# david-gimeno/tailored-avsr

Measured on AMD Instinct MI355X. Metric: utterances/sec fwd+bwd, 12L tailored AV-Branchformer (Conv3d+ResNet-18 lip frontend, fusion, CTC+6L decoder), 4 s clips, batch 32/GPU, higher is better.
Workload: dtype f32

## Files before the change

include/tavsr.h:

```cpp
#ifndef TAVSR_H_
#define TAVSR_H_

#include <stdint.h>

#ifdef __cplusplus
extern "C" {
#endif

typedef void* tavsr_stream_t;

enum { TAVSR_OK = 0, TAVSR_EINVAL = -1, TAVSR_EALIGN = -2, TAVSR_EUNSUPPORTED = -3 };
enum { TAVSR_ACT_NONE = 0, TAVSR_ACT_RELU = 1, TAVSR_ACT_SWISH = 2, TAVSR_ACT_GELU = 3,
       TAVSR_ACT_TANH = 4, TAVSR_ACT_HARDTANH = 5, TAVSR_ACT_SELU = 6 };

int tavsr_version(void);
const char* tavsr_last_error_string(void);

int tavsr_spin(float us, tavsr_stream_t stream);
int tavsr_race_probe(float us, int mode);
int tavsr_stream_create(tavsr_stream_t* out);
int tavsr_probe_launch(int32_t kind, int32_t grid, int32_t block, float* buf, int64_t n, tavsr_stream_t stream);
int tavsr_probe_seam(int32_t kind, int32_t grid, int64_t per_wg, int32_t nphase, float* buf, void* ctl, uint32_t epoch0,
                     tavsr_stream_t stream);
int tavsr_mfma_peak_f32(int32_t iters, int32_t blocks, float* sink, tavsr_stream_t stream);
// ... 314 lines not shown
                         tavsr_stream_t stream);
int tavsr_merge_proj_ok(int32_t T, int32_t D);
int tavsr_merge_proj_fwd(const float* x1, const float* x2, const int64_t* lens, const int64_t* lens2, const float* const* params,
                         const float* w, const float* bias, const float* res, float alpha, float p_drop, const uint64_t* seed_dev,
                         uint64_t drop_offset, float* dots, float* score, float* wout, float* mix, float* out, int32_t B, int32_t T,
                         int32_t D, tavsr_stream_t stream);
int tavsr_merge_proj_fwd_dots(const float* x1, const float* x2, const int64_t* lens, const int64_t* lens2, const float* const* params,
                              const float* w, const float* bias, const float* res, float alpha, float p_drop, const uint64_t* seed_dev,
                              uint64_t drop_offset, const float* rowdots1, const float* rowdots2, float* dots, float* score, float* wout,
                              float* mix, float* out, int32_t B, int32_t T, int32_t D, tavsr_stream_t stream);
int64_t tavsr_merge_bwd_ws(int32_t B, int32_t D);
int tavsr_merge_bwd(const float* dm, const float* x1, const float* x2, const int64_t* lens, const int64_t* lens2,
                    const float* const* params, const float* score, const float* pooled, const float* w,
                    float* dx1, float* dx2, float* const* dparams, int32_t accumulate, float* ws, int32_t B,
                    int32_t T, int32_t D, tavsr_stream_t stream);

int tavsr_conv1_fwd(const float* x, const float* w, const float* bias, float* y, int32_t B, int32_t T,
                    int32_t F, int32_t C, tavsr_stream_t stream);
int64_t tavsr_conv1_bwd_ws(int32_t B, int32_t T, int32_t F, int32_t C);
int tavsr_conv1_bwd(const float* dz, const float* x, float* dw, float* db, int32_t accumulate, float* ws,
                    int32_t B, int32_t T, int32_t F, int32_t C, tavsr_stream_t stream);
int tavsr_im2col3x3s2(const float* y, float* col, int32_t B, int32_t Ti, int32_t Fi, int32_t C,
                      tavsr_stream_t stream);
int tavsr_col2im3x3s2_relu(const float* dcol, const float* yrelu, float* dz, int32_t B, int32_t Ti,
                           int32_t Fi, int32_t C, tavsr_stream_t stream);
int tavsr_transpose_inner(const float* in, float* out, int64_t nb, int32_t R, int32_t Cc, int32_t accumulate,
                          tavsr_stream_t stream);
int tavsr_utterance_mvn(const float* x, const int64_t* lens, float* y, int32_t B, int32_t T, int32_t F,
                        tavsr_stream_t stream);

int64_t tavsr_ctc_loss_ws(int32_t B, int32_t T, int32_t Lmax);
int tavsr_ctc_loss(const float* logits, int64_t ld_t, int64_t ld_b, const int64_t* hlens,
                   const int64_t* targets, int64_t ld_tgt, const int64_t* tlens, int32_t blank,
                   int32_t zero_infinity, float* loss, float* grad, float* ws, int32_t B, int32_t T,
                   int32_t V, int32_t Lmax, tavsr_stream_t stream);
int tavsr_ctc_greedy(const float* logits, int64_t ld_t, int64_t ld_b, const int64_t* hlens, int32_t blank,
                     int64_t* ids, int64_t* hyp, int64_t* hyp_len, int32_t B, int32_t T, int32_t V,
                     tavsr_stream_t stream);
int tavsr_ctc_align_lds_ok(int32_t T, int32_t Lmax);
int64_t tavsr_ctc_align_ws(int32_t N, int32_t T, int32_t Lmax);
int tavsr_ctc_align(const float* logits, int64_t ld_t, int64_t ld_b, const int64_t* hlens, const int32_t* rows,
                    const int64_t* targets, int64_t ld_tgt, const int64_t* tlens, int32_t blank, int64_t* align,
                    float* frame_lp, int32_t* span, float* score, void* ws, int32_t N, int32_t T, int32_t V, int32_t Lmax,
                    tavsr_stream_t stream);

int tavsr_lstm_rows_per_wg(void);
int tavsr_lstm_wt(const float* w_hh, float* w_hh_t, int32_t H, tavsr_stream_t stream);
int tavsr_lstm_fwd(const float* xg, int64_t ld_xg, const float* w_hh_t, const float* b_ih, const float* b_hh,
                   const float* h0, const float* c0, const int64_t* lens, float* y, float* hprev, float* c_all,
                   float* gates, float* hN, float* cN, int32_t B, int32_t L, int32_t H, tavsr_stream_t stream);
int tavsr_lstm_bwd(const float* dy, const float* dhN, const float* dcN, const float* w_hh, const float* c0,
                   const int64_t* lens, const float* c_all, const float* gates, float* dgates, float* dh0, float* dc0,
                   int32_t B, int32_t L, int32_t H, tavsr_stream_t stream);
int tavsr_lstm_step(const float* xg, int64_t ld_xg, const float* w_hh_t, const float* b_ih, const float* b_hh,
                    const float* h_in, const float* c_in, const uint8_t* commit, float* h_out, float* c_out, int32_t N,
                    int32_t H, tavsr_stream_t stream);
int tavsr_rnnt_mask_rows(const float* x, const int64_t* lens, int32_t extra, float* out, int32_t B, int32_t Tn, int32_t D,
                         tavsr_stream_t stream);
int64_t tavsr_rnnt_ws(int32_t B, int32_t T, int32_t U1, int32_t J, int32_t V, int32_t chunk, int32_t grad);
int tavsr_rnnt_joint_rows(const float* e, const float* d, const float* w_out, const float* b_out, const int32_t* y,
                          int64_t ld_y, const int64_t* tlens, const int64_t* ulens, int32_t blank, float* lse,
                          float* lp_blank, float* lp_label, float* ws, int32_t B, int32_t T, int32_t U1, int32_t J,
                          int32_t V, int32_t chunk, tavsr_stream_t stream);
int tavsr_rnnt_lattice_lds_ok(int32_t T, int32_t U1);
int64_t tavsr_rnnt_lattice_ws(int32_t B, int32_t T, int32_t U1);
int tavsr_rnnt_lattice(const float* lp_blank, const float* lp_label, const int64_t* tlens, const int64_t* ulens, float* nll,
                       float* occ, float* p_blank, float* p_label, float* ws, int32_t B, int32_t T, int32_t U1,
                       tavsr_stream_t stream);
int tavsr_rnnt_joint_grad(const float* e, const float* d, const float* w_out, const float* b_out, const int32_t* y,
                          int64_t ld_y, const int64_t* tlens, const int64_t* ulens, int32_t blank, const float* lse,
                          const float* occ, const float* p_blank, const float* p_label, const float* gscale, float inv_b,
                          float* de, float* dd, float* dw_out, float* db_out, float* ws, int32_t B, int32_t T, int32_t U1,
                          int32_t J, int32_t V, int32_t chunk, tavsr_stream_t stream);
int tavsr_rnnt_frame_z(const float* e, const float* d, const int32_t* frame, float* z, int32_t B, int32_t T, int32_t J,
                       tavsr_stream_t stream);
int tavsr_rnnt_greedy_pick(const float* logits, int64_t ldv, const int64_t* tlens, int32_t blank, int32_t* frame,
                           int64_t* tok, uint8_t* commit, int64_t* hyp, int64_t ld_hyp, int32_t* hyp_len, float* score,
                           int32_t B, int32_t V, tavsr_stream_t stream);

int tavsr_rnnt_search_ok(int32_t kind, int32_t K, int32_t V, int32_t T, int32_t u_max, int32_t max_sym_exp);
int64_t tavsr_rnnt_search_ws(int32_t kind, int32_t K, int32_t T, int32_t u_max, int32_t max_sym_exp);
int32_t tavsr_rnnt_search_ws_offset(int32_t kind, int32_t K, int32_t T, int32_t u_max, int32_t max_sym_exp, int32_t which);
int tavsr_rnnt_search_init(int32_t* ws, const int64_t* tlens, int32_t* row_t, int32_t U, int32_t kind, int32_t K, int32_t V,
                           int32_t T, int32_t u_max, int32_t max_sym_exp, tavsr_stream_t stream);
int tavsr_rnnt_search_z(const float* e, const float* d, const int32_t* row_t, float* z, int32_t N, int32_t K, int32_t T,
                        int32_t J, tavsr_stream_t stream);
int tavsr_rnnt_row_topk(const float* logits, int64_t ldv, const int32_t* row_t, float* lp_blank, float* topv, int32_t* topi,
                        int32_t N, int32_t V, int32_t K, tavsr_stream_t stream);
int tavsr_rnnt_gather_state(const float* src_h, const float* src_c, const int32_t* idx, float* dst_h, float* dst_c, int32_t L,
                            int32_t Ns, int32_t Nd, int32_t H, tavsr_stream_t stream);
int tavsr_rnnt_alsd_step(int32_t* ws, const int64_t* tlens, const float* lp_blank, const float* topv, const int32_t* topi,
                         int32_t* row_t, int32_t* parent, int64_t* tok, uint8_t* commit, int32_t U, int32_t K, int32_t V,
                         int32_t T, int32_t u_max, tavsr_stream_t stream);
int tavsr_rnnt_tsd_step(int32_t* ws, const int64_t* tlens, const float* lp_blank, const float* topv, const int32_t* topi,
                        int32_t* row_t, int32_t* parent, int64_t* tok, uint8_t* commit, int32_t* a_src, int32_t* b_sel,
                        int32_t v, int32_t U, int32_t K, int32_t V, int32_t T, int32_t max_sym_exp, tavsr_stream_t stream);

int tavsr_maskctc_init(const float* logits, int64_t ld_t, int64_t ld_b, const int64_t* hlens, int32_t blank,
                       int32_t mask_token, double threshold, int32_t n_iterations, int64_t* y_in, int64_t* y_hat,
                       float* tok_prob, int64_t ld_y, int64_t* y_len, int32_t* plan, int32_t B, int32_t T, int32_t V,
                       tavsr_stream_t stream);
int tavsr_maskctc_step(const float* logits, int64_t ld_l, int64_t ld_b, int64_t* y_in, int64_t ld_y,
                       const int64_t* y_len, const int32_t* plan, int32_t it, int32_t mask_token, int32_t B, int32_t L,
                       int32_t V1, tavsr_stream_t stream);

enum { TAVSR_MASK_UNIFORM_MAX_L = 4096 };
int tavsr_mask_uniform(const int64_t* text, int64_t ld_text, int32_t B, int32_t Lmax, int32_t mask_token, int32_t eos,
                       int32_t ignore_id, const uint64_t* seed_dev, uint64_t offset, int64_t* ys_in, int64_t* ys_out,
                       int64_t ld_y, int32_t* n_target, tavsr_stream_t stream);
int tavsr_count_recip(const int32_t* n, int32_t B, float* inv, tavsr_stream_t stream);

int tavsr_lm_shift(const int64_t* text, int64_t ld_text, const int64_t* lengths, int32_t B, int32_t W, int32_t sos_eos,
                   int64_t* x, int64_t* t, int64_t ld_y, int32_t Wout, int64_t* x_lengths, int32_t* n, tavsr_stream_t stream);
int tavsr_lm_row_sums(const float* x, int64_t ldx, float* out, int32_t rows, int32_t cols, tavsr_stream_t stream);

int tavsr_lsm_loss(const float* logits, int64_t ld, const int64_t* target, int32_t ignore, float smoothing,
                   float* row_loss, float* grad, int32_t* correct, int64_t rows, int32_t V,
                   tavsr_stream_t stream);
int tavsr_embed_pe(const int64_t* ids, const float* table, const float* pe, float scale, float* out, int64_t N,
                   int32_t L, int32_t D, tavsr_stream_t stream);
int tavsr_embed_pe_step(const int64_t* ids, const float* table, const float* pe, float scale, float* out, int64_t N,
                        int32_t L, int32_t D, const int32_t* step_dev, tavsr_stream_t stream);
int tavsr_embed_bwd(const int64_t* ids, const float* dout, float scale, float* dtable, int64_t N, int32_t V,
                    int32_t D, int32_t accumulate, tavsr_stream_t stream);

int tavsr_im2col2d(const float* x, float* col, int64_t N, int32_t H, int32_t W, int32_t C, int32_t KH, int32_t KW,
                   int32_t stride, int32_t pad, tavsr_stream_t stream);
int tavsr_col2im2d(const float* dcol, float* dx, int64_t N, int32_t H, int32_t W, int32_t C, int32_t KH, int32_t KW,
                   int32_t stride, int32_t pad, const float* extra, tavsr_stream_t stream);
int tavsr_im2col_stem(const float* x, float* col, int32_t B, int32_t T, int32_t H, int32_t W, tavsr_stream_t stream);
int64_t tavsr_bn_ws(int64_t M, int32_t C);
int tavsr_bn_stats(const float* x, int64_t M, int32_t C, float eps, float momentum, float* mean, float* var, float* rstd,
                   float* running_mean, float* running_var, int64_t* num_batches_tracked, float* ws, tavsr_stream_t stream);
int tavsr_bn_apply_fwd(const float* x, const float* mean, const float* rstd, const float* gamma, const float* beta,
                       const float* res, float* y, int64_t M, int32_t C, int32_t act, tavsr_stream_t stream);
int tavsr_bn_bwd(const float* dy, const float* x, const float* mean, const float* rstd, const float* gamma, const float* beta,
                 const float* res, float* dz, float* dx, float* dgamma, float* dbeta, int64_t M, int32_t C, int32_t act,
                 float* ws, tavsr_stream_t stream);
int tavsr_bn_bwd_pooled(const float* dpool, const uint8_t* idx, const float* x, const float* mean, const float* rstd,
                        const float* gamma, const float* beta, float* dx, float* dgamma, float* dbeta, int64_t N, int32_t H,
                        int32_t W, int32_t C, int32_t act, float* ws, tavsr_stream_t stream);
int tavsr_rsqrt_eps(const float* v, float eps, float* out, int64_t n, tavsr_stream_t stream);
int tavsr_maxpool3x3s2_fwd(const float* x, float* y, uint8_t* idx, int64_t N, int32_t H, int32_t W, int32_t C,
                           tavsr_stream_t stream);
int tavsr_bn_act_maxpool3x3s2_fwd(const float* x, const float* mean, const float* rstd, const float* gamma, const float* beta,
                                  int32_t act, float* y, uint8_t* idx, int64_t N, int32_t H, int32_t W, int32_t C,
                                  tavsr_stream_t stream);
int tavsr_maxpool3x3s2_bwd(const float* dy, const uint8_t* idx, float* dx, int64_t N, int32_t H, int32_t W, int32_t C,
                           tavsr_stream_t stream);
int tavsr_avgpool_fwd(const float* x, float* y, int64_t N, int32_t P, int32_t C, tavsr_stream_t stream);
int tavsr_avgpool_bwd(const float* dy, float* dx, int64_t N, int32_t P, int32_t C, tavsr_stream_t stream);
int tavsr_fill(float* p, float value, int64_t n, tavsr_stream_t stream);
int tavsr_conv_wflip(const float* w2d, float* wflip, int32_t Cout, int32_t Cin, tavsr_stream_t stream);
int tavsr_copy2d(const float* src, int64_t lds, float* dst, int64_t ldd, int64_t M, int64_t N, tavsr_stream_t stream);

int tavsr_stft_frames(const float* wav, const float* window, float* frames, int32_t B, int64_t N, int32_t T, int32_t n_fft,
                      int32_t hop, int32_t center, tavsr_stream_t stream);
int tavsr_power_spec(const float* spec, int64_t ld_spec, float* P, int32_t ldp, int32_t nfreq, int32_t B, int32_t T,
                     const int64_t* olens, tavsr_stream_t stream);
int tavsr_log_mask(const float* mel, float* out, int32_t B, int32_t T, int32_t n_mels, const int64_t* olens, float floor_,
                   tavsr_stream_t stream);
int tavsr_time_warp(const float* x, float* y, int32_t B, int32_t T, int32_t F, const int64_t* center, const int64_t* warped,
                    const int64_t* lens, tavsr_stream_t stream);
int tavsr_specaug_mask(float* x, int32_t B, int32_t T, int32_t F, const int64_t* fpos, const int64_t* flen, int32_t nf,
                       const int64_t* tpos, const int64_t* tlen, int32_t nt, tavsr_stream_t stream);

int tavsr_rowlin(const float* x, int64_t ldx, const int64_t* gather, const float* gamma, const float* beta, float eps,
                 const float* W, int64_t ldw, const float* bias, int32_t act, const float* res, int64_t ldr,
                 const int64_t* res_gather, float* out, int64_t ldo, int32_t N, int32_t K, int32_t Nout, tavsr_stream_t stream);
int tavsr_rowlin_parts(const float* x, int64_t ldx, int32_t x_parts, int64_t x_pstride, const float* gamma, const float* beta,
                       float eps, const float* W, int64_t ldw, const float* bias, int32_t act, const float* res, int64_t ldr,
                       int32_t res_parts, int64_t res_pstride, float* out, int64_t ldo, int32_t ksplit, int64_t out_pstride,
                       int32_t N, int32_t K, int32_t Nout, tavsr_stream_t stream);
int tavsr_tree_attn_tune(int32_t mode);
int tavsr_rowlin_ok(int32_t N, int32_t K, int32_t with_ln, int32_t ksplit);
int tavsr_tree_attn_step(const float* q, int64_t ldq, const float* kpool, const float* vpool, int64_t ldkv,
                         const int32_t* anc, int64_t ld_anc, int32_t nkeys, float* out, int64_t ldo, int32_t N, int32_t H,
                         int32_t dk, float scale, const int32_t* step_dev, const float* k_new, const float* v_new,
                         int32_t group, tavsr_stream_t stream);
int tavsr_kv_append(const float* k, const float* v, int64_t ld_src, float* kpool, float* vpool, int64_t ldkv, int32_t N,
                    int32_t D, int32_t max_steps, const int32_t* step_dev, tavsr_stream_t stream);
int tavsr_ctc_prefix_step(const float* logp, const int64_t* lens, const float* r_prev, const float* s_prev,
                          const int64_t* last_tok, const int64_t* cand, float* r_new, float* psi, float* psi_abs, float* eos,
                          float* eos_abs, int32_t N, int32_t K, int32_t T, int32_t V, int32_t C, int32_t out_len,
                          int32_t blank, const int32_t* step_dev, tavsr_stream_t stream);
int tavsr_ctc_prefix_step_topk(const float* logp, const int64_t* lens, const float* r_prev, const float* s_prev,
                               const int64_t* last_tok, const float* full, int64_t* cand, float* r_new, float* psi, float* psi_abs,
                               float* eos, float* eos_abs, int32_t N, int32_t K, int32_t T, int32_t V, int32_t C, int32_t out_len,
                               int32_t blank, const int32_t* step_dev, tavsr_stream_t stream);
int tavsr_log_softmax_rows(const float* x, int64_t ldx, float* y, int64_t ldy, int32_t M, int32_t V, float alpha, float add,
                           int32_t accumulate, tavsr_stream_t stream);
int tavsr_beam_combine(const float* full, const int64_t* cand, const float* psi, float* psi_abs, const float* eos_s,
                       const float* eos_abs, const float* s_prev, const float* score, float* weighted, int32_t N, int32_t V,
                       int32_t C, int32_t eos, float w_ctc, tavsr_stream_t stream);
int tavsr_beam_combine_topk(const float* full, const int64_t* cand, const float* psi, float* psi_abs, const float* eos_s,
                            const float* eos_abs, const float* s_prev, const float* score, float* weighted, float* top_s,
                            int64_t* top_i, int32_t N, int32_t K, int32_t V, int32_t C, int32_t eos, float w_ctc,
                            tavsr_stream_t stream);
int tavsr_beam_select_topk(const float* dec, const float* z_lm, float w_lm, float add, const float* psi_all, float* psi_abs_all,
                           const float* eos_s, const float* eos_abs, const float* s_prev, const float* score, float* full_out,
                           float* weighted, int64_t* cand_out, float* top_s, int64_t* top_i, int32_t N, int32_t K, int32_t V,
                           int32_t C, int32_t eos, float w_ctc, tavsr_stream_t stream);
int tavsr_beam_reorder(const int64_t* top_i, const float* top_s, const int64_t* cand, const float* r_new, const float* psi_abs,
                       const int64_t* yseq, const int32_t* anc, float* r_out, float* s_out, int64_t* yseq_out, int32_t* anc_out,
                       int64_t* tok_out, float* score_out, int32_t N, int32_t K, int32_t V, int32_t C, int32_t T, int32_t ld_y,
                       int32_t ld_a, const int32_t* step_dev, int32_t* hist, int32_t hist_steps, tavsr_stream_t stream);
int tavsr_beam_reorder_begin(const int64_t* top_i, const float* top_s, const int64_t* cand, const float* r_new, const float* psi_abs,
                             const int64_t* yseq, const int32_t* anc, float* r_out, float* s_out, int64_t* yseq_out, int32_t* anc_out,
                             int64_t* tok_out, float* score_out, int32_t N, int32_t K, int32_t V, int32_t C, int32_t T, int32_t ld_y,
                             int32_t ld_a, const int32_t* step_dev, int32_t* hist, int32_t hist_steps, const int32_t* maxlen,
                             int32_t eos, tavsr_stream_t stream);
int tavsr_beam_step_begin(float* score, const int64_t* tok, int32_t* anc, int32_t ld_a, const int32_t* maxlen, int32_t N, int32_t K,
                          int32_t eos, const int32_t* step_dev, tavsr_stream_t stream);
int tavsr_ctc_beam_search_ok(int32_t K, int32_t V, int32_t T);
int tavsr_ctc_beam_search(const float* logp, const int64_t* lens, const int32_t* maxlen, int32_t* hist, int32_t* n_steps, int32_t U,
                          int32_t K, int32_t T, int32_t V, int32_t hist_steps, int32_t sos, int32_t eos, int32_t blank, float w_ctc,
                          float add, int32_t end_detect, float d_end, tavsr_stream_t stream);
int tavsr_timesync_ok(int32_t K, int32_t V, int32_t T, int32_t C);
int64_t tavsr_timesync_ws(int32_t K, int32_t V, int32_t T, int32_t C);
int32_t tavsr_timesync_ws_offset(int32_t K, int32_t V, int32_t T, int32_t C, int32_t which);
int tavsr_timesync_init(int32_t* ws, int64_t* tok, int32_t* pos, int32_t* nkeys, int32_t* anc, int64_t ld_anc, int32_t* frame_dev,
                        int32_t U, int32_t K, int32_t V, int32_t T, int32_t C, int32_t sos, int32_t blank, tavsr_stream_t stream);
int tavsr_timesync_step(const float* lpz, const int64_t* lens, int32_t* ws, const float* dec_new, float* dec_rows,
                        const float* lm_new, float* lm_rows, int64_t* tok, int32_t* pos, int32_t* nkeys, int32_t* anc,
                        int32_t* anc_tmp, int64_t ld_anc, const int32_t* frame_dev, int32_t U, int32_t K, int32_t V, int32_t T,
                        int32_t C, int32_t sos, int32_t blank, float w_ctc, float w_dec, float w_lm, float pen,
                        tavsr_stream_t stream);
int tavsr_timesync_search(const float* lpz, const int64_t* lens, int32_t* ws, int32_t U, int32_t K, int32_t V, int32_t T, int32_t C,
                          int32_t sos, int32_t blank, float w_ctc, float pen, tavsr_stream_t stream);
int tavsr_tree_attn_rows(const float* q, int64_t ldq, const float* kpool, const float* vpool, int64_t ldkv, const int32_t* anc,
                         int64_t ld_anc, const int32_t* nkeys_row, int32_t max_keys, float* out, int64_t ldo, int32_t N, int32_t H,
                         int32_t dk, float scale, const float* k_new, const float* v_new, tavsr_stream_t stream);
int tavsr_embed_pe_rows(const int64_t* ids, const float* table, const float* pe, float scale, float* out, int64_t N, int32_t L,
                        int32_t D, const int32_t* pos, tavsr_stream_t stream);
enum { TAVSR_NGRAM_MAX_ORDER = 8 };
int tavsr_ngram_score(const int32_t* word, const float* logp, const float* backoff, const int32_t* child_begin, int32_t n_unigrams,
                      int32_t order, int32_t bos_word, float unk_logp, const int32_t* word_map, const int64_t* yseq, int64_t ld_y,
                      int32_t L, int32_t step, const int32_t* step_dev, const int64_t* cand, int32_t C, float alpha, float add,
                      int32_t accumulate, float* out, int64_t ldo, int32_t N, int32_t V, tavsr_stream_t stream);
int tavsr_act_fwd(const float* x, float* y, int64_t n, int32_t act, tavsr_stream_t stream);

int tavsr_adam_step(float* p, const float* g, float* m, float* v, int64_t n, float lr, float beta1, float beta2, float eps,
                    int64_t step, float grad_scale, tavsr_stream_t stream);
int tavsr_adamw_step(float* p, const float* g, float* m, float* v, int64_t n, float lr, float beta1, float beta2, float eps,
                     float weight_decay, int64_t step, float grad_scale, tavsr_stream_t stream);

int tavsr_bucket_copy(float* const* ptrs_dev, const int64_t* off_dev, const int64_t* n_dev, int32_t ntensors, float* flat,
                      float scale, int32_t to_flat, int64_t max_n, tavsr_stream_t stream);

int tavsr_dp_unique_id(void* id128);
int tavsr_dp_init(int32_t rank, int32_t nranks, const void* id128);
int32_t tavsr_dp_world(void);
int tavsr_dp_allreduce(float* flat, int64_t n, tavsr_stream_t stream);
int tavsr_dp_broadcast(float* flat, int64_t n, int32_t root, tavsr_stream_t stream);
int tavsr_dp_destroy(void);

int tavsr_multi_add(float* const* dst, const float* const* src, const int64_t* n, int32_t ntensors, tavsr_stream_t stream);
int tavsr_multi_copy(void* const* dst, const void* const* src, const int64_t* nbytes, int32_t nbuffers, tavsr_stream_t stream);
int tavsr_multi_copy_inc(void* const* dst, const void* const* src, const int64_t* nbytes, int32_t nbuffers, int64_t* counters,
                         int32_t ncounters, tavsr_stream_t stream);

int tavsr_dropout(const float* x, float* y, int64_t n, float p, const uint64_t* seed_dev, uint64_t offset,
                  tavsr_stream_t stream);
int tavsr_rng_advance(uint64_t* seed_dev, tavsr_stream_t stream);
int tavsr_rng_step(uint64_t* seed_dev, uint64_t* step_seed_dev, tavsr_stream_t stream);
int tavsr_dropout_add(const float* a, const float* t, float* y, int64_t n, float p, float alpha, const uint64_t* seed_dev,
                      uint64_t offset, tavsr_stream_t stream);
int tavsr_dropout_act_bwd(const float* dh, const float* z, float* dz, int64_t n, float p, int32_t act,
                          const uint64_t* seed_dev, uint64_t offset, tavsr_stream_t stream);

int tavsr_edit_distance(const int32_t* ref, const int64_t* ref_off, const int32_t* hyp, const int64_t* hyp_off, int32_t n_pairs,
                        int32_t max_len, int32_t* dist, tavsr_stream_t stream);
int tavsr_bootstrap_rates(const int32_t* dist, const int32_t* reflen, int32_t n, int32_t iters, uint64_t seed, double* rates,
                          tavsr_stream_t stream);

int tavsr_video_prep(const void* src, int32_t is_u8, int32_t Ts, int32_t H, int32_t W, const int32_t* frames, int32_t T,
                     int32_t y0, int32_t x0, int32_t th, int32_t tw, int32_t flip, const float* mean, const float* std,
                     int32_t n_affine, const uint8_t* masked, float* mean_frame_ws, float* dst, int32_t Tpad, float pad,
                     tavsr_stream_t stream);
int tavsr_add_noise(const float* audio, const float* noise, float* out, int64_t n, float inv_snr, tavsr_stream_t stream);
int64_t tavsr_resample_len(int64_t n_in, double factor);
int tavsr_resample_sinc(const float* x, int64_t n_in, float* y, int64_t n_out, double factor, double rolloff, int32_t zeros, double beta,
                        tavsr_stream_t stream);

#ifdef __cplusplus
}
#endif
#endif
```

tailored-avsr_amd/csrc/gemm_conv.hip:

```cpp
#include <algorithm>
#include <vector>

#include "gemm_glds.h"

namespace tavsr {

constexpr int kOrdRuns = 80;
struct TileOrder {
  int nruns;
  int start[kOrdRuns];
  int cum[kOrdRuns + 1];
  int w[kOrdRuns];
};

__host__ __device__ inline void tile_order_map(const TileOrder& o, int b, int tiles_m, int tiles_n, int& mt, int& nt) {
  const int per = 8 * tiles_n;
  const int g = b / per, j = b - g * per, s0 = 8 * g;
  int r0 = 0;
  while (r0 + 1 < o.nruns && o.cum[r0 + 1] <= s0) ++r0;
  bool uniform = s0 + 8 <= tiles_m;
  if (uniform) {
    int r7 = r0;
    while (r7 + 1 < o.nruns && o.cum[r7 + 1] <= s0 + 7) ++r7;
    uniform = o.w[r7] == o.w[r0];
  }
  const int s = s0 + (uniform ? (j & 7) : j / tiles_n);
  nt = uniform ? (j >> 3) : j % tiles_n;
  int r = r0;
  while (r + 1 < o.nruns && o.cum[r + 1] <= s) ++r;
  mt = o.start[r] + s - o.cum[r];
}

__host__ __device__ inline int dw_tile_order(int q, int tiles_m, int tiles_n, int H, int W) {
  if (tiles_n % 9 != 0) return q;
  const int tpt = tiles_n / 9, per = tiles_m * tpt;
  const int rank = q / per, rem = q - rank * per;
  const unsigned long long taps = (H - 1) * W >= H * (W - 1) ? 0x862053714ull : 0x862071534ull;
  const int tap = (int)((taps >> (4 * rank)) & 15);
  return (rem / tpt) * tiles_n + tap * tpt + rem % tpt;
}

__host__ __device__ inline void dw_xcd_order(int j, int tiles_m, int tiles_n, int ns, int& zs, int& q) {
  const int tiles = tiles_m * tiles_n;
  zs = j / tiles;
  q = j - zs * tiles;
  if (tiles_n % 9 != 0) return;
  const int per = tiles_m * (tiles_n / 9);
  const int rank = j / (ns * per), rem = j - rank * (ns * per);
  zs = rem / per;
  q = rank * per + rem - zs * per;
}

struct ConvGeom {
  int cs, p0, Ho, Wo;
  bool c9;
  __device__ __forceinline__ explicit ConvGeom(const tavsr_gemm_desc& d) {
    cs = d.conv_stride > 1 ? d.conv_stride : 1;
    c9 = d.conv_taps != 1;
    p0 = d.conv_taps == 90 ? 1 : 0;
    Ho = (d.conv_H - 1 - 2 * p0) / cs + 1;
    Wo = (d.conv_W - 1 - 2 * p0) / cs + 1;
  }
};

template <int BM, int NT>
struct ImageRows {
  using L = GLoader<BM, false, NT>;
  int64_t off[L::NR];
  uint32_t mask[L::NR];
  __device__ __forceinline__ void issue(const TileCtx& c, bool c9, int kk, int tap, float* img) const {
    const tavsr_gemm_desc& d = c.d;
    const int toff = c9 ? (tap / 3 - 1) * d.conv_W + (tap % 3 - 1) : 0;
    const int64_t delta = (int64_t)toff * d.conv_C + (kk - tap * d.conv_C);
#pragma unroll
    for (int i = 0; i < L::NR; ++i)
      dma16(((mask[i] >> tap) & 1u) ? c.A + off[i] + delta : d.conv_zero, img + (i * NT + c.wave * 64) * 4);
  }
};

template <int BM, int NT>
struct ConvRowsA {
  using R = ImageRows<BM, NT>;
  static constexpr int kDma = R::L::NR;
  const TileCtx& c;
  bool c9;
  R rows;
  __device__ __forceinline__ explicit ConvRowsA(const TileCtx& c_) : c(c_) {
    const tavsr_gemm_desc& d = c.d;
    const ConvGeom g(d);
    c9 = g.c9;
    R::L::offsets(d.lda, c.m0, d.M, c.tid, rows.off);
#pragma unroll
    for (int i = 0; i < R::L::NR; ++i) {
      const int m = min(c.m0 + ((i * NT + c.tid) >> 3), d.M - 1);
      const int x = (m % g.Wo) * g.cs + g.p0, y = ((m / g.Wo) % g.Ho) * g.cs + g.p0;
      if (g.cs > 1 || g.p0) rows.off[i] += ((int64_t)((m / (g.Wo * g.Ho)) * d.conv_H + y) * d.conv_W + x - m) * d.conv_C;
      uint32_t mk = 0;
#pragma unroll
      for (int tap = 0; tap < 9; ++tap)
        mk |= (uint32_t)((unsigned)(y + tap / 3 - 1) < (unsigned)d.conv_H && (unsigned)(x + tap % 3 - 1) < (unsigned)d.conv_W) << tap;
      rows.mask[i] = g.c9 ? mk : 1u;
    }
  }
  __device__ __forceinline__ void issue(int kt, float* img) {
    const int kk = c.kbeg + kt * kBK;
    rows.issue(c, c9, kk, kk / c.d.conv_C, img);
  }
};
template <int BM, int BN, int NT, bool BKM>
struct SourceFor<1, false, BM, BN, NT, false, BKM> {
  using type = PairSource<ConvRowsA<BM, NT>, PlainOperand<BN, BKM, NT, true>, BM>;
};

template <int BM, int BN, int NT, bool BKM>
struct PosMajorRowsSource : SourceDefaults {
  using R = ImageRows<BM, NT>;
  using LB = GLoader<BN, BKM, NT>;
  static constexpr int kDma = R::L::NR + LB::NR;
  static constexpr bool kPosMajorRows = true;
  const TileCtx& c;
  PosMajor pm{};
  uint32_t taps = 0;
  int tap, cb, nk;
  bool c9;
  R rows;
  int64_t offB[LB::NR];
  __device__ __forceinline__ explicit PosMajorRowsSource(const TileCtx& c_) : c(c_) {
    const tavsr_gemm_desc& d = c.d;
    const ConvGeom g(d);
    c9 = g.c9;
    LB::offsets(d.ldb, c.n0, d.N, c.tid, offB);
    pm.H = g.Ho; pm.W = g.Wo;
    pm.st = g.cs; pm.HI = d.conv_H; pm.WI = d.conv_W;
    pm.n = d.M / (g.Ho * g.Wo);
    const int vlo = c.m0 / pm.n, vhi = min(c.m0 + BM - 1, d.M - 1) / pm.n;
    for (int v = vlo; v <= vhi; ++v) {
      int y, x;
      pm.pos(v, y, x);
      taps |= pm.taps(y, x);
      pm.rp = y * g.Wo + x;
    }
    pm.uni = vlo == vhi;
    pm.base = vlo * pm.n;
    nk = 0;
    for (int t = 0; t < 9; ++t) {
      const int lo = max(c.kbeg, t * d.conv_C), hi = min(c.kend, (t + 1) * d.conv_C);
      if (((taps >> t) & 1u) && hi > lo) nk += (hi - lo) / kBK;
    }
    tap = c.kbeg / d.conv_C;
    cb = (c.kbeg - tap * d.conv_C) / kBK;
    if (!((taps >> tap) & 1u)) {
      const uint32_t up = taps >> (tap + 1) << (tap + 1);
      tap = up ? __builtin_ctz(up) : 9;
      cb = 0;
    }
#pragma unroll
    for (int i = 0; i < R::L::NR; ++i) {
      const int q = i * NT + c.tid, row = q >> 3;
      const int r = min(c.m0 + row, d.M - 1);
      int y, x, img;
      if (pm.uni) {
        y = pm.rp / g.Wo; x = pm.rp - y * g.Wo; img = r - pm.base;
      } else {
        const int v = r / pm.n;
        pm.pos(v, y, x);
        img = r - v * pm.n;
      }
      rows.off[i] = ((int64_t)img * (d.conv_H * d.conv_W) + g.cs * y * d.conv_W + g.cs * x) * d.lda + ((q & 7) ^ ((row >> 1) & 7)) * 4;
      rows.mask[i] = pm.taps(y, x);
    }
  }
  __device__ __forceinline__ int steps() const { return nk; }
  __device__ __forceinline__ const PosMajor* row_map() const { return &pm; }
  __device__ __forceinline__ void issue(int, float* stage) {
    const tavsr_gemm_desc& d = c.d;
    const int ktap = tap, kk = tap * d.conv_C + cb * kBK;
    const int wrap = (cb + 1) * kBK >= d.conv_C;
    const uint32_t up = taps >> (tap + 1) << (tap + 1);
    cb = wrap ? 0 : cb + 1;
    tap = !wrap ? tap : up ? __builtin_ctz(up) : 9;
    rows.issue(c, c9, kk, ktap, stage);
    LB::issue(c.B + (BKM ? (int64_t)kk * d.ldb : kk), offB, stage + BM * kBK, c.wave);
  }
};
template <int BM, int BN, int NT, bool BKM>
struct SourceFor<1, true, BM, BN, NT, false, BKM> {
  using type = PosMajorRowsSource<BM, BN, NT, BKM>;
};

template <int BN, int NT>
struct PatchB {
  using L = GLoader<BN, true, NT>;
  static constexpr int kDma = L::NR;
  const TileCtx& c;
  const ConvGeom g;
  int ox[L::NR], oy[L::NR], img[L::NR];
  int sb, salo, sahi, tapoff, cb, dy, dx;
  __device__ __forceinline__ explicit PatchB(const TileCtx& c_) : c(c_), g(c_.d) {
    const tavsr_gemm_desc& d = c.d;
    const int sa = kBK / g.Wo;
    sb = kBK - sa * g.Wo;
    sahi = sa / g.Ho;
    salo = sa - sahi * g.Ho;
    const int tap = c.n0 / d.conv_C;
    cb = c.n0 - tap * d.conv_C;
    dy = g.c9 ? tap / 3 - 1 : 0;
    dx = g.c9 ? tap % 3 - 1 : 0;
    tapoff = dy * d.conv_W + dx;
#pragma unroll
    for (int i = 0; i < L::NR; ++i) {
      const int m = c.kbeg + (i * NT + c.tid) / (BN / 4);
      const int t = m / g.Wo;
      ox[i] = m - t * g.Wo;
      img[i] = t / g.Ho;
      oy[i] = t - img[i] * g.Ho;
    }
  }
  __device__ __forceinline__ void issue(int, float* dst) {
    const tavsr_gemm_desc& d = c.d;
#pragma unroll
    for (int i = 0; i < L::NR; ++i) {
      const int r = (((i * NT + c.tid) % (BN / 4)) * 4);
      const int x = ox[i] * g.cs + g.p0, y = oy[i] * g.cs + g.p0;
      const bool ok = (unsigned)(y + dy) < (unsigned)d.conv_H && (unsigned)(x + dx) < (unsigned)d.conv_W;
      const int64_t pix = (int64_t)(img[i] * d.conv_H + y) * d.conv_W + x;
      dma16(ok ? c.B + (pix + tapoff) * d.conv_C + cb + r : d.conv_zero, dst + (i * NT + c.wave * 64) * 4);
      int nx = ox[i] + sb;
      const int w1 = nx >= g.Wo ? 1 : 0;
      nx -= w1 ? g.Wo : 0;
      int ny = oy[i] + salo + w1;
      const int w2 = ny >= g.Ho ? 1 : 0;
      ny -= w2 ? g.Ho : 0;
      ox[i] = nx; oy[i] = ny; img[i] += sahi + w2;
    }
  }
};
template <int BM, int BN, int NT>
struct SourceFor<2, false, BM, BN, NT, true, true> {
  using type = PairSource<PlainOperand<BM, true, NT, false>, PatchB<BN, NT>, BM>;
};

template <int BM, int BN, int NT>
struct PatchWalkSource : SourceDefaults {
  using LA = GLoader<BM, true, NT>;
  using LB = GLoader<BN, true, NT>;
  static constexpr int kDma = LA::NR + LB::NR;
  const TileCtx& c;
  const ConvGeom g;
  int64_t offA[LA::NR];
  int tapoff, cb, dy, dx;
  int n, i0, nk;
  int v = 0, img = 0, x = 0, y = 0;
  __device__ __forceinline__ static int rowsum_n0(const tavsr_gemm_desc& d) { return 4 * d.conv_C; }
  __device__ __forceinline__ bool ok(int py, int px) const {
    return (unsigned)(g.cs * py + dy) < (unsigned)c.d.conv_H && (unsigned)(g.cs * px + dx) < (unsigned)c.d.conv_W;
  }
  __device__ __forceinline__ explicit PatchWalkSource(const TileCtx& c_) : c(c_), g(c_.d) {
    const tavsr_gemm_desc& d = c.d;
    const int tap = c.n0 / d.conv_C;
    cb = c.n0 - tap * d.conv_C;
    dy = g.c9 ? tap / 3 - 1 : 0;
    dx = g.c9 ? tap % 3 - 1 : 0;
    tapoff = dy * d.conv_W + dx;
    const int P = g.Ho * g.Wo;
    i0 = c.kbeg / P;
    n = (c.kend - c.kbeg) / P;
    LA::offsets(d.lda, c.m0, d.M, c.tid, offA);
#pragma unroll
    for (int i = 0; i < LA::NR; ++i) offA[i] -= (int64_t)((i * NT + c.tid) / (BM / 4)) * d.lda;
    if (n % kBK == 0) {
      int ny = 0, nx = 0;
      for (int py = 0; py < g.Ho; ++py) ny += (unsigned)(g.cs * py + dy) < (unsigned)d.conv_H;
      for (int px = 0; px < g.Wo; ++px) nx += (unsigned)(g.cs * px + dx) < (unsigned)d.conv_W;
      nk = (n / kBK) * ny * nx;
    } else {
      nk = 0;
      int prev = 0, py = 0, px = 0;
      for (int pv = 0; pv < P; ++pv) {
        if (ok(py, px)) {
          const int s_lo = max(pv * n / kBK, prev), s_hi = ((pv + 1) * n - 1) / kBK + 1;
          if (s_hi > s_lo) { nk += s_hi - s_lo; prev = s_hi; }
        }
        if (++px == g.Wo) { px = 0; ++py; }
      }
    }
  }
  __device__ __forceinline__ int steps() const { return nk; }
  __device__ __forceinline__ void advance() {
    img += kBK;
    while (img >= n) {
      img -= n;
      ++v;
      if (++x == g.Wo) { x = 0; ++y; }
    }
  }
  __device__ __forceinline__ int64_t locate(int kl, int& py, int& px, int& pimg) const {
    int pv = v;
    pimg = img + kl;
    py = y; px = x;
    while (pimg >= n) {
      pimg -= n;
      ++pv;
      if (++px == g.Wo) { px = 0; ++py; }
    }
    pimg += i0;
    return (int64_t)pimg * (g.Ho * g.Wo) + pv;
  }
  __device__ __forceinline__ void issue(int, float* stage) {
    const tavsr_gemm_desc& d = c.d;
    for (;;) {
      bool any = false;
      int end = img + kBK, py = y, px = x;
      for (;;) {
        any |= ok(py, px);
        if (end <= n) break;
        end -= n;
        if (++px == g.Wo) { px = 0; ++py; }
      }
      if (any) break;
      advance();
    }
#pragma unroll
    for (int i = 0; i < LA::NR; ++i) {
      int py, px, pimg;
      const int64_t pix = locate((i * NT + c.tid) / (BM / 4), py, px, pimg);
      dma16(c.A + pix * d.lda + offA[i], stage + (i * NT + c.wave * 64) * 4);
    }
#pragma unroll
    for (int i = 0; i < LB::NR; ++i) {
      const int r = (((i * NT + c.tid) % (BN / 4)) * 4);
      int py, px, pimg;
      locate((i * NT + c.tid) / (BN / 4), py, px, pimg);
      const int64_t pix = ((int64_t)pimg * d.conv_H + g.cs * py) * d.conv_W + g.cs * px;
      dma16(ok(py, px) ? c.B + (pix + tapoff) * d.conv_C + cb + r : d.conv_zero, stage + BM * kBK + (i * NT + c.wave * 64) * 4);
    }
    advance();
  }
};
template <int BM, int BN, int NT>
struct SourceFor<2, true, BM, BN, NT, true, true> {
// ... 80 lines not shown
    const int ft = m / (g.Wo * g.Ho);
    t = ft % g.T;
    off = (ft * g.H + 2 * ho) * g.W + 2 * wo;
    th = frame_row_ok();
  }
  __device__ __forceinline__ void issue(int, float* img) {
#pragma unroll
    for (int i = 0; i < kDma; ++i) {
      const bool ok = th && (unsigned)(2 * wo + c3) < (unsigned)g.W;
      dma4(ok ? c.B + (off + tapoff) : c.d.conv_zero, img + i * NT + c.wave * 64);
      wo += 4;
      off += 8;
      if (wo >= g.Wo) {
        wo -= g.Wo;
        off += g.W;
        if (++ho == g.Ho) {
          ho = 0;
          if (++t == g.T) t = 0;
        }
        th = frame_row_ok();
      }
    }
  }
};
template <int BM, int BN, int NT>
struct SourceFor<5, false, BM, BN, NT, true, true> {
  using type = PairSource<PlainOperand<BM, true, NT, false>, Stem5B<BN, NT>, BM>;
};

struct PaddedStemGeom {
  int Hp, Wp, Tp, Ho, Wo, T;
  __device__ __forceinline__ explicit PaddedStemGeom(const tavsr_gemm_desc& d)
      : Hp(d.conv_H), Wp(d.conv_W), Tp(d.conv_C), Ho((d.conv_H - 6) / 2), Wo((d.conv_W - 8) / 2), T(d.conv_C - 5) {}
  __device__ __forceinline__ int pixel(int m) const {
    const int wo = m % Wo, ho = (m / Wo) % Ho, ft = m / (Wo * Ho);
    return (((ft / T) * Tp + ft % T) * Hp + 2 * ho) * Wp + 2 * wo;
  }
};

template <int BM, int NT>
struct Stem6A {
  using L = GLoader<BM, false, NT>;
  static constexpr int kDma = L::NR;
  const TileCtx& c;
  const PaddedStemGeom g;
  int base[L::NR], cl[L::NR];
  __device__ __forceinline__ explicit Stem6A(const TileCtx& c_) : c(c_), g(c_.d) {
#pragma unroll
    for (int i = 0; i < L::NR; ++i) {
      const int q = i * NT + c.tid, row = q >> 3;
      cl[i] = (q & 7) ^ ((row >> 1) & 7);
      base[i] = g.pixel(min(c.m0 + row, c.d.M - 1));
    }
  }
  __device__ __forceinline__ void issue(int kt, float* img) {
#pragma unroll
    for (int i = 0; i < L::NR; ++i) {
      const int ch = (c.kbeg >> 2) + kt * 8 + cl[i], r = ch >> 1, a = r / 7, b = r - 7 * a;
      dma16(c.A + (base[i] + (a * g.Hp + b) * g.Wp + 4 * (ch & 1)), img + (i * NT + c.wave * 64) * 4);
    }
  }
};
template <int BM, int BN, int NT>
struct SourceFor<6, false, BM, BN, NT, false, false> {
  using type = PairSource<Stem6A<BM, NT>, PlainOperand<BN, false, NT, true>, BM>;
};

template <int BN, int NT>
struct Stem7B {
  using L = GLoader<BN, true, NT>;
  static constexpr int kDma = L::NR;
  const TileCtx& c;
  const PaddedStemGeom g;
  int wo[L::NR], ho[L::NR], t[L::NR], off[L::NR];
  int tapoff;
  __device__ __forceinline__ explicit Stem7B(const TileCtx& c_) : c(c_), g(c_.d) {
    constexpr int CPR = BN / 4;
    int ch = (c.n0 >> 2) + (c.tid % CPR);
    if (ch >= 72) ch = 0;
    const int r = ch >> 1, a = r / 7, b = r - 7 * a;
    tapoff = (a * g.Hp + b) * g.Wp + 4 * (ch & 1);
#pragma unroll
    for (int i = 0; i < L::NR; ++i) {
      const int m = c.kbeg + (i * NT + c.tid) / CPR;
      wo[i] = m % g.Wo; ho[i] = (m / g.Wo) % g.Ho; t[i] = (m / (g.Wo * g.Ho)) % g.T;
      off[i] = g.pixel(m);
    }
  }
  __device__ __forceinline__ void issue(int, float* img) {
    constexpr int STEP = 32;
#pragma unroll
    for (int i = 0; i < L::NR; ++i) {
      dma16(c.B + (off[i] + tapoff), img + (i * NT + c.wave * 64) * 4);
      wo[i] += STEP;
      off[i] += 2 * STEP;
      while (wo[i] >= g.Wo) {
        wo[i] -= g.Wo;
        off[i] += 2 * g.Wp - 2 * g.Wo;
        if (++ho[i] == g.Ho) {
          ho[i] = 0;
          off[i] += (g.Hp - 2 * g.Ho) * g.Wp;
          if (++t[i] == g.T) { t[i] = 0; off[i] += (g.Tp - g.T) * g.Hp * g.Wp; }
        }
      }
    }
  }
};
template <int BM, int BN, int NT>
struct SourceFor<7, false, BM, BN, NT, true, true> {
  using type = PairSource<PlainOperand<BM, true, NT, false>, Stem7B<BN, NT>, BM>;
};

struct GemmArgsOrd {
  GemmArgs g;
  TileOrder ord;
};
template <int CONV, bool PM>
struct TileMap<CONV, PM, true> {
  __device__ __forceinline__ static const GemmArgs& map(const GemmArgsOrd& x, int& bid, int& zidx) {
    bid = xcd_remap(blockIdx.x, gridDim.x);
    zidx = blockIdx.z;
    if (x.ord.nruns > 0) {
      int mt, nt;
      tile_order_map(x.ord, blockIdx.x, x.g.tiles_m, x.g.tiles_n, mt, nt);
      bid = mt * x.g.tiles_n + nt;
    }
    return x.g;
  }
  __device__ __forceinline__ static const GemmArgs& map(const GemmArgs& args, int& bid, int& zidx) {
    bid = xcd_remap(blockIdx.x, gridDim.x);
    zidx = blockIdx.z;
    if (args.zmap) {
      const int tiles = gridDim.x, l = blockIdx.x + tiles * blockIdx.z, j = l >> 3;
      int zs = j / tiles;
      bid = j % tiles;
      if constexpr (PM && CONV == 2) {
        if (!(args.d.conv_posmajor & 2)) {
          if (args.n_big > 0) dw_xcd_order(j, args.tiles_m, args.tiles_n, args.nsplit >> 3, zs, bid);
          bid = dw_tile_order(bid, args.tiles_m, args.tiles_n, args.d.conv_H, args.d.conv_W);
        }
      }
      zidx = (l & 7) + 8 * zs;
    }
    return args;
  }
};

static int conv_ho(const tavsr_gemm_desc& d) { return (d.conv_H - 1) / std::max(d.conv_stride, 1) + 1; }
static int conv_wo(const tavsr_gemm_desc& d) { return (d.conv_W - 1) / std::max(d.conv_stride, 1) + 1; }

constexpr int kPmStride2MaxPos = 36;
static bool conv_pm(const tavsr_gemm_desc& d) {
  const bool stride_ok = d.conv_stride <= 1 || (d.conv_stride == 2 && (d.conv_posmajor & 8) && conv_ho(d) * conv_wo(d) <= kPmStride2MaxPos);
  return d.conv_posmajor && (d.conv_mode == 1 || d.conv_mode == 2) && stride_ok && (d.conv_taps == 0 || d.conv_taps == 9) &&
         (d.conv_mode == 2 || !d.a_rowsum);
}

static void tile_order_build(const tavsr_gemm_desc& d, int BM, int nsplit, TileOrder& o) {
  o.nruns = 0;
  const int cs = std::max(d.conv_stride, 1);
  const int P = conv_ho(d) * conv_wo(d);
  if (nsplit != 1 || (d.conv_posmajor & 2) || P <= 0 || d.M < P) return;
  struct Key { int H, W, cs, M, BM; };
  static thread_local Key last{0, 0, 0, 0, 0};
  static thread_local TileOrder last_o;
  if (last.H == d.conv_H && last.W == d.conv_W && last.cs == cs && last.M == d.M && last.BM == BM) { o = last_o; return; }
  PosMajor pm{};
  pm.H = conv_ho(d); pm.W = conv_wo(d); pm.n = d.M / P;
  pm.st = cs; pm.HI = d.conv_H; pm.WI = d.conv_W;
  std::vector<uint32_t> tp(P);
  for (int v = 0; v < P; ++v) {
    int y, x;
    pm.pos(v, y, x);
    tp[v] = pm.taps(y, x);
  }
  struct Run { int start, len, w; };
  std::vector<Run> runs;
  const int tiles_m = cdiv(d.M, BM);
  for (int i = 0; i < tiles_m; ++i) {
    const int vlo = (int)((int64_t)i * BM / pm.n);
    const int vhi = std::min((int)(std::min<int64_t>((int64_t)i * BM + BM - 1, d.M - 1) / pm.n), P - 1);
    uint32_t mk = 0;
    for (int v = vlo; v <= vhi; ++v) mk |= tp[v];
    const int w = __builtin_popcount(mk);
    if (!runs.empty() && runs.back().w == w) ++runs.back().len;
    else runs.push_back(Run{i, 1, w});
    if ((int)runs.size() > kOrdRuns) return;
  }
  std::stable_sort(runs.begin(), runs.end(), [](const Run& a, const Run& b) { return a.w > b.w; });
  int cum = 0;
  for (size_t r = 0; r < runs.size(); ++r) {
    o.start[r] = runs[r].start; o.cum[r] = cum; o.w[r] = runs[r].w;
    cum += runs[r].len;
  }
  o.cum[runs.size()] = cum;
  o.nruns = (int)runs.size();
  last = Key{d.conv_H, d.conv_W, cs, d.M, BM};
  last_o = o;
}

template <int BM, int BN, int MINW, bool AK, bool BKM, int CONV, bool PM>
static int launch_conv_tile(const tavsr_gemm_desc& d, const Plan& p, hipStream_t s) {
  const int zmap = (CONV == 2 || CONV == 5 || CONV == 7) && p.nsplit >= 8 && p.nsplit % 8 == 0;
  const bool two = PM && CONV == 2;
  GemmArgs a{d, p.kchunk, p.nsplit, cdiv(d.M, BM), cdiv(d.N, BN), (int)vec_epi_ok(d), zmap, two ? p.n_big : 0, two ? p.kunit : 0};
  const dim3 grid(a.tiles_m * a.tiles_n, 1, p.nsplit);
  if constexpr (PM && CONV == 1) {
    GemmArgsOrd ao{a, {}};
    tile_order_build(d, BM, p.nsplit, ao.ord);
    hipLaunchKernelGGL((gemm_glds_kernel<BM, BN, 2, 2, 2, MINW, AK, BKM, 1, CONV, true>), grid, dim3(256), 0, s, ao);
  } else {
    hipLaunchKernelGGL((gemm_glds_kernel<BM, BN, 2, 2, 2, MINW, AK, BKM, 1, CONV, PM>), grid, dim3(256), 0, s, a);
  }
  TAVSR_LAUNCH_CHECK();
  return launch_epilogue(a, s);
}

template <int BM, int BN, int MINW, bool AK, bool BKM, int CONV>
static int launch_conv_pm(const tavsr_gemm_desc& d, const Plan& p, hipStream_t s) {
  return conv_pm(d) ? launch_conv_tile<BM, BN, MINW, AK, BKM, CONV, true>(d, p, s) : launch_conv_tile<BM, BN, MINW, AK, BKM, CONV, false>(d, p, s);
}

int launch_conv(const tavsr_gemm_desc& d, const Plan& p, hipStream_t s) {
  switch (d.conv_mode) {
    case 1:
      if (d.b_kmajor) return launch_conv_pm<64, 64, 5, false, true, 1>(d, p, s);
      if (p.nsplit == 1 && d.N % 128 == 0) return launch_conv_pm<64, 128, 3, false, false, 1>(d, p, s);
      return launch_conv_pm<64, 64, 5, false, false, 1>(d, p, s);
    case 2:
      if (d.M % 128 == 0) return launch_conv_pm<128, 64, 3, true, true, 2>(d, p, s);
      return launch_conv_pm<64, 64, 5, true, true, 2>(d, p, s);
    case 4: return launch_conv_tile<64, 64, 5, false, false, 4, false>(d, p, s);
    case 5: return launch_conv_tile<64, 64, 5, true, true, 5, false>(d, p, s);
    case 6: return launch_conv_tile<64, 64, 5, false, false, 6, false>(d, p, s);
    default: return launch_conv_tile<64, 64, 5, true, true, 7, false>(d, p, s);
  }
}

Plan plan_conv(const tavsr_gemm_desc& d, bool can_split, int force_split) {
  Plan pc = plan(d, can_split, true);
  if ((d.conv_mode == 2 || d.conv_mode == 5 || d.conv_mode == 7) && can_split) {
    const bool wide = d.conv_mode == 2 && d.M % 128 == 0;
    const long tiles = (long)cdiv(d.M, wide ? 128 : 64) * cdiv(d.N, 64);
    constexpr long target64 = 2560L;
    constexpr long target128 = 2304L;
    const long target = wide ? target128 : target64;
    int unit = 32;
    if (conv_pm(d)) {
      const int P = conv_ho(d) * conv_wo(d);
      int g = P, b = 32;
      while (b) { const int t = g % b; g = b; b = t; }
      unit = P / g * 32;
      if (pc.nsplit > 1) {
        pc.kchunk = cdiv(pc.kchunk, unit) * unit;
        pc.nsplit = cdiv(d.K, pc.kchunk);
      }
    }
    const long want = std::min<long>(std::max<long>(1, target / tiles), d.K / 512);
    if (want > pc.nsplit) {
      pc.kchunk = cdiv(cdiv(d.K, want), unit) * unit;
      pc.nsplit = cdiv(d.K, pc.kchunk);
    }
    if (pc.nsplit >= 16 && pc.nsplit % 8 != 0) {
      for (long w8 = pc.nsplit / 8 * 8; w8 >= 8; w8 -= 8) {
        const int kc = cdiv(cdiv(d.K, w8), unit) * unit;
        if (cdiv(d.K, kc) % 8 == 0) { pc.kchunk = kc; pc.nsplit = cdiv(d.K, kc); break; }
        if (w8 < pc.nsplit / 2) break;
      }
    }
    if (conv_pm(d) && d.conv_mode == 2 && !(d.conv_posmajor & 4) && d.K % unit == 0) {
      const long U = d.K / unit, round4 = (wide ? 768 : 1280) / 4;
      const long w = std::min<long>(force_split > 0 ? force_split : want, U) / 8 * 8;
      const bool missed = target - (long)pc.nsplit * tiles > round4, hits = target - w * tiles <= round4;
      if (w >= 8 && U % w != 0 && (force_split > 0 || (missed && hits))) {
        pc.nsplit = (int)w;
        pc.kchunk = (int)(U / w) * unit;
        pc.n_big = (int)(U % w);
        pc.kunit = unit;
      }
    }
  }
  return pc;
}

}

extern "C" int tavsr_conv_tile_order(int H, int W, int images, int bm, int tiles_n, int32_t* tile_m, int32_t* tile_n, int max_blocks) {
  using namespace tavsr;
  if (H <= 0 || W <= 0 || images <= 0 || bm <= 0 || tiles_n <= 0) return 0;
  tavsr_gemm_desc d{};
  d.conv_H = H; d.conv_W = W; d.M = images * H * W; d.conv_posmajor = 1;
  TileOrder o;
  tile_order_build(d, bm, 1, o);
  if (o.nruns == 0) return 0;
  const int tiles_m = cdiv(d.M, bm), nwg = tiles_m * tiles_n;
  for (int b = 0; b < nwg && b < max_blocks; ++b) tile_order_map(o, b, tiles_m, tiles_n, tile_m[b], tile_n[b]);
  return nwg;
}

extern "C" int tavsr_conv_dw_tile_order(int H, int W, int tiles_m, int tiles_n, int32_t* tile, int max_tiles) {
  if (H <= 0 || W <= 0 || tiles_m <= 0 || tiles_n <= 0) return 0;
  for (int q = 0; q < tiles_m * tiles_n && q < max_tiles; ++q) tile[q] = tavsr::dw_tile_order(q, tiles_m, tiles_n, H, W);
  return tiles_m * tiles_n;
}

extern "C" int tavsr_conv_dw_plan(int H, int W, int cin, int cout, int images, int posmajor, int force_split, int32_t* out) {
  using namespace tavsr;
  if (H <= 0 || W <= 0 || cin <= 0 || cout <= 0 || images <= 0 || !out) return 0;
  tavsr_gemm_desc d{};
  d.conv_mode = 2; d.conv_H = H; d.conv_W = W; d.conv_C = cin; d.conv_stride = 1; d.conv_taps = 9; d.conv_posmajor = posmajor;
  d.M = cout; d.N = 9 * cin; d.K = images * H * W; d.a_kmajor = d.b_kmajor = 1; d.nb1 = d.nb2 = 1;
  const Plan p = plan_conv(d, true, force_split);
  out[0] = p.kchunk; out[1] = p.n_big; out[2] = p.kunit;
  return p.nsplit;
}

extern "C" int tavsr_conv_dw_xcd_order(int H, int W, int tiles_m, int tiles_n, int ns, int32_t* slice, int32_t* tile, int max_tiles) {
  if (H <= 0 || W <= 0 || tiles_m <= 0 || tiles_n <= 0 || ns <= 0) return 0;
  for (int j = 0; j < ns * tiles_m * tiles_n && j < max_tiles; ++j) {
    int zs, q;
    tavsr::dw_xcd_order(j, tiles_m, tiles_n, ns, zs, q);
    slice[j] = zs;
    tile[j] = tavsr::dw_tile_order(q, tiles_m, tiles_n, H, W);
  }
  return ns * tiles_m * tiles_n;
}

#ifdef TAVSR_GEMM_TRACE
namespace tavsr {
int conv_trace_read(unsigned long long* out, int max_rows) { return trace_read_unit(out, max_rows); }
}
#endif
```

tailored-avsr_amd/csrc/gemm_glds.h:

```cpp
#pragma once
#include <type_traits>

#include "common.h"

namespace tavsr {

typedef float f32x16 __attribute__((ext_vector_type(16)));
constexpr int kBK = 32;

struct GemmArgs {
  tavsr_gemm_desc d;
  int kchunk;
  int nsplit;
  int tiles_m, tiles_n;
  int vec_epi;
  int zmap;
  int n_big, kunit;
};

template <int ROWS, int BK, bool KMAJOR>
struct Tile {
  static constexpr int LD = KMAJOR ? (ROWS + 4) : (BK + 4);
  static constexpr int SIZE = KMAJOR ? BK * LD : ROWS * LD;
};
// ... 203 lines not shown
                                                int tid, int zidx, const PosMajor* pm = nullptr) {
  __syncthreads();
#pragma unroll
  for (int i = 0; i < TM; ++i)
#pragma unroll
    for (int j = 0; j < TN; ++j)
#pragma unroll
      for (int r = 0; r < 16; ++r)
        img[(wm * TM * 32 + i * 32 + (r & 3) + 8 * (r >> 2) + 4 * lk) * BN + wn * TN * 32 + j * 32 + lr] = acc[i][j][r];
  __syncthreads();
  constexpr int V4R = BN / 4, PER = BM * BN / 4 / NT;
  static_assert(BM * BN % (4 * NT) == 0, "tile must divide over the block");
  const bool split = nsplit > 1;
  float* base;
  int64_t ld;
  if (split) {
    base = d.ws + ((int64_t)zidx * gridDim.y + blockIdx.y) * ((int64_t)d.M * d.N);
    ld = d.N;
  } else {
    base = d.C + coff;
    ld = d.ldc;
  }
  const float* R = (!split && d.R) ? d.R + z1 * d.sR1 + z2 * d.sR2 : nullptr;
  float* Z = (!split && d.Z) ? d.Z + coff : nullptr;
  const float* DZ = (!split && d.DZ) ? d.DZ + coff : nullptr;
  const bool rowstat = BN == 64 && !split && d.rowstat != nullptr;
#pragma unroll
  for (int q = 0; q < PER; ++q) {
    const int idx = q * NT + tid, row = idx / V4R, c4 = idx % V4R;
    const int mv = m0 + row, n = n0 + 4 * c4;
    const bool ok = mv < d.M && n < d.N;
    const int m = PM && ok ? pm->row(mv) : mv;
    float4 v = make_float4(0.f, 0.f, 0.f, 0.f);
    if (ok) {
    v = *reinterpret_cast<const float4*>(img + row * BN + 4 * c4);
    const int64_t o = (int64_t)m * ld + n;
    if (!split) {
      if (d.bias) {
        const float4 b = *reinterpret_cast<const float4*>(d.bias + n);
        v.x += b.x; v.y += b.y; v.z += b.z; v.w += b.w;
      }
      if (Z) *reinterpret_cast<float4*>(Z + o) = v;
      v.x = act_fwd(d.act, v.x); v.y = act_fwd(d.act, v.y); v.z = act_fwd(d.act, v.z); v.w = act_fwd(d.act, v.w);
      if (DZ) {
        const float4 z = *reinterpret_cast<const float4*>(DZ + o);
        v.x *= act_bwd(d.dact, z.x); v.y *= act_bwd(d.dact, z.y); v.z *= act_bwd(d.dact, z.z); v.w *= act_bwd(d.dact, z.w);
      }
      if (d.drop_p > 0.f) {
        const uint64_t sd = d.drop_seed[0], ctr = (d.drop_offset >> 2) + (uint64_t)(((int64_t)m * d.N + n) >> 2);
        const uint32_t thr = (uint32_t)((double)d.drop_p * 4294967296.0);
        const float ik = 1.f / (1.f - d.drop_p);
        uint32_t w[4];
        philox4x32_10((uint32_t)ctr, (uint32_t)(ctr >> 32), 0u, 0u, (uint32_t)sd, (uint32_t)(sd >> 32), w);
        v.x = w[0] >= thr ? v.x * ik : 0.f; v.y = w[1] >= thr ? v.y * ik : 0.f;
        v.z = w[2] >= thr ? v.z * ik : 0.f; v.w = w[3] >= thr ? v.w * ik : 0.f;
      }
      v.x *= d.alpha; v.y *= d.alpha; v.z *= d.alpha; v.w *= d.alpha;
      if (R) {
        const float4 rr = *reinterpret_cast<const float4*>(R + (int64_t)m * d.ldr + n);
        v.x += rr.x; v.y += rr.y; v.z += rr.z; v.w += rr.w;
      }
    }
    *reinterpret_cast<float4*>(base + o) = v;
    }
    if (rowstat) {
      float s1 = ok ? (v.x + v.y) + (v.z + v.w) : 0.f, s2 = 0.f;
      if (d.rowdot_a) {
        const float4 wa = ok ? *reinterpret_cast<const float4*>(d.rowdot_a + n) : make_float4(0.f, 0.f, 0.f, 0.f);
        const float4 wb = ok ? *reinterpret_cast<const float4*>(d.rowdot_b + n) : make_float4(0.f, 0.f, 0.f, 0.f);
        s1 = (v.x * wa.x + v.y * wa.y) + (v.z * wa.z + v.w * wa.w);
        s2 = (v.x * wb.x + v.y * wb.y) + (v.z * wb.z + v.w * wb.w);
      }
#pragma unroll
      for (int o2 = 8; o2 > 0; o2 >>= 1) s1 += __shfl_xor(s1, o2, 64);
      if (!d.rowdot_a && ok) {
        const float tm = s1 / (float)min(64, d.N - n0);
        const float e0 = v.x - tm, e1 = v.y - tm, e2 = v.z - tm, e3 = v.w - tm;
        s2 = (e0 * e0 + e1 * e1) + (e2 * e2 + e3 * e3);
      }
#pragma unroll
      for (int o2 = 8; o2 > 0; o2 >>= 1) s2 += __shfl_xor(s2, o2, 64);
      if (c4 == 0 && mv < d.M)
        *reinterpret_cast<float2*>(d.rowstat + ((int64_t)m * ((d.N + 63) / 64) + n0 / 64) * 2) = make_float2(s1, s2);
    }
  }
}

static bool aligned16(const void* p) { return (reinterpret_cast<uintptr_t>(p) & 15) == 0; }
static bool vec_epi_ok(const tavsr_gemm_desc& d) {
  return d.N % 4 == 0 && d.ldc % 4 == 0 && d.sC1 % 4 == 0 && d.sC2 % 4 == 0 && aligned16(d.C) && (!d.bias || aligned16(d.bias)) &&
         (!d.Z || aligned16(d.Z)) && (!d.DZ || aligned16(d.DZ)) &&
         (!d.R || (aligned16(d.R) && d.ldr % 4 == 0 && d.sR1 % 4 == 0 && d.sR2 % 4 == 0)) && (!d.ws || aligned16(d.ws));
}

typedef __attribute__((address_space(3))) float lds_float;
typedef const __attribute__((address_space(1))) float glb_float;

template <int ROWS, bool KMAJOR, int NT>
struct GLoader {
  static constexpr int NR = ROWS * 8 / NT;
  static_assert(ROWS * 8 % NT == 0, "tile must divide over the block");
  __device__ static __forceinline__ void offsets(int64_t ld, int row0, int nrows, int tid, int64_t (&off)[NR]) {
#pragma unroll
    for (int i = 0; i < NR; ++i) {
      const int q = i * NT + tid;
      if (KMAJOR) {
        const int k = q / (ROWS / 4);
        int r = row0 + (q % (ROWS / 4)) * 4;
        if (r + 3 >= nrows) r = row0;
        off[i] = (int64_t)k * ld + r;
      } else {
        const int row = q >> 3, cp = q & 7;
        const int cl = cp ^ ((row >> 1) & 7);
        off[i] = (int64_t)min(row0 + row, nrows - 1) * ld + cl * 4;
      }
    }
  }
  __device__ static __forceinline__ void issue(const float* __restrict__ g, const int64_t (&off)[NR],
                                               float* __restrict__ stage, int wave) {
#pragma unroll
    for (int i = 0; i < NR; ++i)
      __builtin_amdgcn_global_load_lds((glb_float*)(g + off[i]), (lds_float*)(stage + (i * NT + wave * 64) * 4), 16, 0, 0);
  }
};

__device__ __forceinline__ void dma16(const float* src, float* dst) {
  __builtin_amdgcn_global_load_lds((glb_float*)src, (lds_float*)dst, 16, 0, 0);
}
__device__ __forceinline__ void dma4(const float* src, float* dst) {
  __builtin_amdgcn_global_load_lds((glb_float*)src, (lds_float*)dst, 4, 0, 0);
}

#ifndef TAVSR_GEMM_SB
#define TAVSR_GEMM_SB 1
#endif
#if TAVSR_GEMM_SB
#define GEMM_SB() __builtin_amdgcn_sched_barrier(0)
#else
#define GEMM_SB()
#endif

template <int ROWS, bool KMAJOR>
__device__ __forceinline__ void read_frag_g(const float* __restrict__ s, int row, int g, int lk, float (&f)[4]) {
  if (KMAJOR) {
    const float* p = s + (g * 8 + 4 * lk) * ROWS + row;
#pragma unroll
    for (int j = 0; j < 4; ++j) f[j] = p[j * ROWS];
  } else {
    const float4 v = *reinterpret_cast<const float4*>(s + row * 32 + (((2 * g + lk) ^ ((row >> 1) & 7)) << 2));
    f[0] = v.x; f[1] = v.y; f[2] = v.z; f[3] = v.w;
  }
}

template <int N>
__device__ __forceinline__ void wait_vmcnt() {
  asm volatile("s_waitcnt vmcnt(%0)" ::"n"(N) : "memory");
}

#ifdef TAVSR_GEMM_TRACE
constexpr int kTraceMax = 1 << 15;
static __device__ unsigned long long g_trace[kTraceMax][6];
static __device__ unsigned int g_trace_n;
#define TAVSR_TRACE_DECL unsigned long long tr_t[4], tr_c[4]; tr_t[0] = wall_clock64(); tr_t[1] = tr_t[0]; tr_c[1] = tr_c[2] = 0;
#define TAVSR_TRACE_AT(i) { tr_t[i] = wall_clock64(); tr_c[i] = __builtin_readcyclecounter(); }
static int trace_read_unit(unsigned long long* out, int max_rows) {
  unsigned int n = 0;
  if (hipDeviceSynchronize() != hipSuccess) return -1;
  if (hipMemcpyFromSymbol(&n, HIP_SYMBOL(g_trace_n), sizeof(n)) != hipSuccess) return -1;
  int rows = (int)(n < (unsigned)kTraceMax ? n : kTraceMax);
  if (rows > max_rows) rows = max_rows;
  if (rows > 0 && hipMemcpyFromSymbol(out, HIP_SYMBOL(g_trace), (size_t)rows * 6 * sizeof(unsigned long long)) != hipSuccess) return -1;
  n = 0;
  if (hipMemcpyToSymbol(HIP_SYMBOL(g_trace_n), &n, sizeof(n)) != hipSuccess) return -1;
  return rows;
}
int conv_trace_read(unsigned long long* out, int max_rows);
#else
#define TAVSR_TRACE_DECL
#define TAVSR_TRACE_AT(i)
#endif

struct TileCtx {
  const tavsr_gemm_desc& d;
  const float* A;
  const float* B;
  int m0, n0;
  int kbeg, kend;
  int tid, wave;
};

struct SourceDefaults {
  static constexpr bool kPosMajorRows = false;
  __device__ __forceinline__ const PosMajor* row_map() const { return nullptr; }
  __device__ __forceinline__ static int rowsum_n0(const tavsr_gemm_desc&) { return 0; }
  __device__ __forceinline__ void fix_last(float*, int, int, int) const {}
};

template <int ROWS, bool KMAJOR, int NT, bool B_SIDE>
struct PlainOperand {
  using L = GLoader<ROWS, KMAJOR, NT>;
  static constexpr int kDma = L::NR;
  const TileCtx& c;
  int64_t off[L::NR];
  const float* gk;
  int64_t kstep;
  __device__ __forceinline__ explicit PlainOperand(const TileCtx& c_) : c(c_) {
    const int64_t ld = B_SIDE ? c.d.ldb : c.d.lda;
    L::offsets(ld, B_SIDE ? c.n0 : c.m0, B_SIDE ? c.d.N : c.d.M, c.tid, off);
    kstep = KMAJOR ? (int64_t)kBK * ld : kBK;
    gk = (B_SIDE ? c.B : c.A) + (KMAJOR ? (int64_t)c.kbeg * ld : c.kbeg);
  }
  __device__ __forceinline__ void issue(int kt, float* img) { L::issue(gk + kt * kstep, off, img, c.wave); }
};

template <class HA, class HB, int BM>
struct PairSource : SourceDefaults {
  static constexpr int kDma = HA::kDma + HB::kDma;
  HA a;
  HB b;
  int nk;
  __device__ __forceinline__ explicit PairSource(const TileCtx& c) : a(c), b(c), nk((c.kend - c.kbeg) / kBK) {}
  __device__ __forceinline__ int steps() const { return nk; }
  __device__ __forceinline__ void issue(int kt, float* stage) {
    a.issue(kt, stage);
    b.issue(kt, stage + BM * kBK);
  }
};

template <int CONV, bool PM, int BM, int BN, int NT, bool AK, bool BKM>
struct SourceFor;
template <int BM, int BN, int NT, bool AK, bool BKM>
struct SourceFor<0, false, BM, BN, NT, AK, BKM> {
  using type = PairSource<PlainOperand<BM, AK, NT, false>, PlainOperand<BN, BKM, NT, true>, BM>;
};

template <int BM, int BN, int WM, int WN, int S, bool AK, bool BKM, int KW = 1, int CONV = 0, bool PM = false>
__device__ __forceinline__ void glds_tile(const tavsr_gemm_desc& d, int kchunk, int nsplit, int tiles_n, int bid, bool vec_epi,
                                          int zidx, int n_big = 0, int kunit = 0) {
  constexpr int BK = kBK, NG = BK / 8;
  static_assert(NG % KW == 0, "k-groups must divide over the wave sets");
  static_assert(!PM || KW == 1, "position-major order: one wave set");
  constexpr int NT = WM * WN * KW * 64;
  constexpr int TM = BM / WM / 32, TN = BN / WN / 32;
  using Src = typename SourceFor<CONV, PM, BM, BN, NT, AK, BKM>::type;
  constexpr int ASZ = BM * BK, STAGE = (BM + BN) * BK;
  constexpr int G = Src::kDma;
  static_assert((S - 2) * G <= 63, "vmcnt field");
  __shared__ __attribute__((aligned(1024))) float smem[S * STAGE];

  const int tid = threadIdx.x;
  const int lane = tid & 63;
  const int wave = __builtin_amdgcn_readfirstlane(tid >> 6);
  const int kw = wave / (WM * WN), w2 = wave % (WM * WN);
  const int wm = w2 / WN, wn = w2 % WN;
  const int lr = lane & 31, lk = lane >> 5;

  TAVSR_TRACE_DECL
  const int m0 = (bid / tiles_n) * BM;
  const int n0 = (bid % tiles_n) * BN;
  const int z1 = blockIdx.y / d.nb2, z2 = blockIdx.y % d.nb2;
  const float* A = d.A + z1 * d.sA1 + z2 * d.sA2;
  const float* B = d.B + z1 * d.sB1 + z2 * d.sB2;
  const int64_t coff = z1 * d.sC1 + z2 * d.sC2;

  f32x16 acc[TM][TN];
#pragma unroll
  for (int i = 0; i < TM; ++i)
#pragma unroll
    for (int j = 0; j < TN; ++j)
#pragma unroll
      for (int r = 0; r < 16; ++r) acc[i][j][r] = 0.f;
  float asum[TM];
#pragma unroll
  for (int i = 0; i < TM; ++i) asum[i] = 0.f;
  float bpre[TN];
#pragma unroll
  for (int j = 0; j < TN; ++j) {
    const int n = n0 + wn * TN * 32 + j * 32 + lr;
    bpre[j] = (d.bias && nsplit == 1 && n < d.N) ? d.bias[n] : 0.f;
  }

  const int kbeg = zidx * kchunk + min(zidx, n_big) * kunit;
  const int kend = min(d.K, kbeg + kchunk + (zidx < n_big ? kunit : 0));
  const TileCtx ctx{d, A, B, m0, n0, kbeg, kend, tid, wave};
  Src src(ctx);
  const int nk = src.steps();
  const bool want_rowsum = d.a_rowsum != nullptr && n0 == Src::rowsum_n0(d) && wn == 0;

  const int arow = wm * TM * 32 + lr, brow = wn * TN * 32 + lr;
  auto compute = [&](int st) {
    const float* a_s = smem + st * STAGE;
    const float* b_s = a_s + ASZ;
    float af[2][TM][4], bf[2][TN][4];
#pragma unroll
    for (int i = 0; i < TM; ++i) read_frag_g<BM, AK>(a_s, arow + i * 32, kw, lk, af[0][i]);
#pragma unroll
    for (int j = 0; j < TN; ++j) read_frag_g<BN, BKM>(b_s, brow + j * 32, kw, lk, bf[0][j]);
#pragma unroll
    for (int q = 0; q < NG / KW; ++q) {
      const int c = q & 1;
      if (q + 1 < NG / KW) {
#pragma unroll
        for (int i = 0; i < TM; ++i) read_frag_g<BM, AK>(a_s, arow + i * 32, kw + (q + 1) * KW, lk, af[c ^ 1][i]);
#pragma unroll
        for (int j = 0; j < TN; ++j) read_frag_g<BN, BKM>(b_s, brow + j * 32, kw + (q + 1) * KW, lk, bf[c ^ 1][j]);
      }
      GEMM_SB();
#pragma unroll
      for (int kk = 0; kk < 4; ++kk)
#pragma unroll
        for (int i = 0; i < TM; ++i)
#pragma unroll
          for (int j = 0; j < TN; ++j)
            acc[i][j] = __builtin_amdgcn_mfma_f32_32x32x2f32(af[c][i][kk], bf[c][j][kk], acc[i][j], 0, 0, 0);
#pragma unroll
      for (int i = 0; i < TM; ++i) asum[i] += (af[c][i][0] + af[c][i][1]) + (af[c][i][2] + af[c][i][3]);
      GEMM_SB();
    }
  };

#pragma unroll
  for (int j = 0; j < S - 1; ++j)
    if (j < nk) src.issue(j, smem + j * STAGE);
  int st = 0;
  int kt = 0;
  for (; kt + S - 1 < nk; ++kt) {
    wait_vmcnt<(S - 2) * G>();
    __builtin_amdgcn_s_barrier();
#ifdef TAVSR_GEMM_TRACE
    if (kt == 0) TAVSR_TRACE_AT(1)
#endif
    const int sn = st == 0 ? S - 1 : st - 1;
    src.issue(kt + S - 1, smem + sn * STAGE);
    compute(st);
    st = st + 1 == S ? 0 : st + 1;
  }
  for (; kt < nk; ++kt) {
    wait_vmcnt<0>();
    __builtin_amdgcn_s_barrier();
    if (kt == nk - 1 && ((kend - kbeg) & 3) != 0) src.fix_last(smem + st * STAGE, kend - kbeg, kt, tid);
    compute(st);
    st = st + 1 == S ? 0 : st + 1;
  }
  TAVSR_TRACE_AT(2)
  if (KW > 1) {
    constexpr int PER = TM * TN * 16;
    float* red = smem;
    float* rsum = smem + (KW - 1) * WM * WN * PER * 64;
    static_assert(((KW - 1) * WM * WN * (PER + TM) * 64) <= S * STAGE, "reduction must fit in the staging ring");
    __syncthreads();
    if (kw > 0) {
      float* r0 = red + ((kw - 1) * WM * WN + w2) * PER * 64 + lane;
#pragma unroll
      for (int i = 0; i < TM; ++i)
#pragma unroll
        for (int j = 0; j < TN; ++j)
#pragma unroll
          for (int r = 0; r < 16; ++r) r0[((i * TN + j) * 16 + r) * 64] = acc[i][j][r];
#pragma unroll
      for (int i = 0; i < TM; ++i) rsum[(((kw - 1) * WM * WN + w2) * TM + i) * 64 + lane] = asum[i];
    }
    __syncthreads();
    if (kw > 0) return;
#pragma unroll
    for (int s2 = 0; s2 < KW - 1; ++s2) {
      const float* r0 = red + (s2 * WM * WN + w2) * PER * 64 + lane;
#pragma unroll
      for (int i = 0; i < TM; ++i)
#pragma unroll
        for (int j = 0; j < TN; ++j)
#pragma unroll
          for (int r = 0; r < 16; ++r) acc[i][j][r] += r0[((i * TN + j) * 16 + r) * 64];
#pragma unroll
      for (int i = 0; i < TM; ++i) asum[i] += rsum[((s2 * WM * WN + w2) * TM + i) * 64 + lane];
    }
  }
  if (KW == 1 && vec_epi) {
    static_assert(KW > 1 || BM * BN <= S * STAGE, "the output tile image must fit in the staging ring");
    if (want_rowsum) {
#pragma unroll
      for (int i = 0; i < TM; ++i) asum[i] += __shfl_xor(asum[i], 32, 64);
      if (lk == 0) {
#pragma unroll
        for (int i = 0; i < TM; ++i) {
          const int m = m0 + wm * TM * 32 + i * 32 + lr;
          if (m < d.M) {
            if (nsplit > 1) (d.ws + (int64_t)nsplit * gridDim.y * d.M * d.N)[(int64_t)zidx * d.M + m] = asum[i];
            else d.a_rowsum[m] = d.alpha * asum[i];
          }
        }
      }
    }
    finish_tile_vec<BM, BN, NT, TM, TN, Src::kPosMajorRows>(d, nsplit, acc, smem, m0, n0, wm, wn, lr, lk, z1, z2, coff, tid, zidx, src.row_map());
  } else {
    finish_tile<TM, TN, Src::kPosMajorRows>(d, nsplit, acc, asum, want_rowsum, m0, n0, wm, wn, lr, lk, z1, z2, coff, zidx, bpre, src.row_map());
  }
#ifdef TAVSR_GEMM_TRACE
  __builtin_amdgcn_s_waitcnt(0);
  TAVSR_TRACE_AT(3)
  if (tid == 0) {
    unsigned int slot = atomicAdd(&g_trace_n, 1u);
    if (slot < (unsigned)kTraceMax) {
      for (int i = 0; i < 4; ++i) g_trace[slot][i] = tr_t[i];
      g_trace[slot][4] = ((unsigned long long)__builtin_amdgcn_s_getreg((31 << 11) | 20) << 32) | __builtin_amdgcn_s_getreg((31 << 11) | 4);
      g_trace[slot][5] = ((tr_c[2] - tr_c[1]) & 0xFFFFFFFFFFull) | ((unsigned long long)nk << 40);
    }
  }
#endif
}

__device__ __forceinline__ int xcd_remap(int bid, int nwg) {
  const int xcd = bid & 7, q = nwg >> 3, r = nwg & 7;
  return (xcd < r ? xcd * (q + 1) : r * (q + 1) + (xcd - r) * q) + (bid >> 3);
}

struct GemmArgsOrd;
template <int CONV, bool PM, bool CONV_LAUNCH = (CONV != 0 && CONV != 3)>
struct TileMap;
template <int CONV, bool PM>
struct TileMap<CONV, PM, false> {
  __device__ __forceinline__ static const GemmArgs& map(const GemmArgs& args, int& bid, int& zidx) {
    bid = xcd_remap(blockIdx.x, gridDim.x);
    zidx = blockIdx.z;
    return args;
  }
};

template <int BM, int BN, int WM, int WN, int S, int MINW, bool AK, bool BKM, int KW = 1, int CONV = 0, bool PM = false>
__global__ __launch_bounds__(WM* WN * KW * 64, MINW)
void gemm_glds_kernel(const std::conditional_t<PM && CONV == 1, GemmArgsOrd, GemmArgs> xargs) {
  int bid, zidx;
  const GemmArgs& args = TileMap<CONV, PM>::map(xargs, bid, zidx);
  glds_tile<BM, BN, WM, WN, S, AK, BKM, KW, CONV, PM>(args.d, args.kchunk, args.nsplit, args.tiles_n, bid, args.vec_epi != 0, zidx,
                                                      args.n_big, args.kunit);
}

template <typename F>
static int launch_layout(const tavsr_gemm_desc& d, F&& f) {
  if (!d.a_kmajor && !d.b_kmajor) return f(std::false_type{}, std::false_type{});
  if (!d.a_kmajor && d.b_kmajor) return f(std::false_type{}, std::true_type{});
  if (d.a_kmajor && d.b_kmajor) return f(std::true_type{}, std::true_type{});
  return f(std::true_type{}, std::false_type{});
}

struct Plan {
  int cfg, nsplit, kchunk;
  int n_big = 0, kunit = 0;
};
Plan plan(const tavsr_gemm_desc& d, bool allow_split, bool fast);
int launch_epilogue(const GemmArgs& a, hipStream_t s);
Plan plan_conv(const tavsr_gemm_desc& d, bool can_split, int force_split = 0);
int launch_conv(const tavsr_gemm_desc& d, const Plan& p, hipStream_t s);

}
```

tailored-avsr_amd/csrc/vision.hip:

```cpp
#include <float.h>

#include <algorithm>

#include "common.h"

namespace tavsr {

__global__ void im2col2d_kernel(const float* __restrict__ x, float* __restrict__ col, int H, int W, int Ho, int Wo,
                                int C4, int KH, int KW, int stride, int pad, int64_t total4) {
  const int64_t i = (int64_t)blockIdx.x * blockDim.x + threadIdx.x;
  if (i >= total4) return;
  const int c4 = (int)(i % C4);
  int64_t r = i / C4;
  const int k = (int)(r % (KH * KW));
  const int64_t m = r / (KH * KW);
  const int wo = (int)(m % Wo), ho = (int)((m / Wo) % Ho);
  const int64_t n = m / ((int64_t)Wo * Ho);
  const int h = ho * stride - pad + k / KW, w = wo * stride - pad + k % KW;
  float4 v = make_float4(0.f, 0.f, 0.f, 0.f);
  if (h >= 0 && h < H && w >= 0 && w < W) v = reinterpret_cast<const float4*>(x)[((n * H + h) * W + w) * C4 + c4];
  reinterpret_cast<float4*>(col)[i] = v;
}

__global__ void col2im2d_kernel(const float* __restrict__ dcol, float* __restrict__ dx, int H, int W, int Ho, int Wo,
                                int C4, int KH, int KW, int stride, int pad, int64_t total4, const float* __restrict__ extra) {
  const int64_t i = (int64_t)blockIdx.x * blockDim.x + threadIdx.x;
  if (i >= total4) return;
  const int c4 = (int)(i % C4);
  int64_t r = i / C4;
  const int w = (int)(r % W), h = (int)((r / W) % H);
  const int64_t n = r / ((int64_t)W * H);
  float4 acc = make_float4(0.f, 0.f, 0.f, 0.f);
  for (int kh = 0; kh < KH; ++kh) {
    const int hn = h + pad - kh;
    if (hn < 0 || hn % stride) continue;
    const int ho = hn / stride;
    if (ho >= Ho) continue;
    for (int kw = 0; kw < KW; ++kw) {
      const int wn = w + pad - kw;
      if (wn < 0 || wn % stride) continue;
      const int wo = wn / stride;
      if (wo >= Wo) continue;
      const float4 v = reinterpret_cast<const float4*>(dcol)[(((n * Ho + ho) * Wo + wo) * (KH * KW) + kh * KW + kw) * C4 + c4];
      acc.x += v.x; acc.y += v.y; acc.z += v.z; acc.w += v.w;
    }
  }
  if (extra && h % stride == 0 && w % stride == 0 && h / stride < Ho && w / stride < Wo) {
    const float4 v = reinterpret_cast<const float4*>(extra)[((n * Ho + h / stride) * Wo + w / stride) * C4 + c4];
    acc.x += v.x; acc.y += v.y; acc.z += v.z; acc.w += v.w;
  }
  reinterpret_cast<float4*>(dx)[i] = acc;
}

constexpr int kStemLd = 104;
__global__ __launch_bounds__(256) void im2col_stem_kernel(const float* __restrict__ x, float* __restrict__ col, int T, int H, int W,
                                                          int Ho, int Wo) {
  __shared__ float rows[35][kStemLd];
  const int ho = blockIdx.x % Ho, bt = blockIdx.x / Ho;
  const int t = bt % T;
  const float* xb = x + (int64_t)(bt - t) * H * W;
  for (int e = threadIdx.x; e < 35 * kStemLd; e += 256) {
    const int r = e / kStemLd, cix = e % kStemLd;
    const int kt = r / 7, kh = r % 7;
    const int tt = t - 2 + kt, h = ho * 2 - 3 + kh, w = cix - 3;
    float v = 0.f;
    if ((unsigned)tt < (unsigned)T && (unsigned)h < (unsigned)H && (unsigned)w < (unsigned)W) v = xb[((int64_t)tt * H + h) * W + w];
    rows[r][cix] = v;
  }
  __syncthreads();
  float4* out = reinterpret_cast<float4*>(col) + (int64_t)blockIdx.x * Wo * 64;
  for (int e = threadIdx.x; e < Wo * 64; e += 256) {
    const int wo = e >> 6, k4 = e & 63;
    float v[4];
#pragma unroll
    for (int j = 0; j < 4; ++j) {
      const int k = k4 * 4 + j;
      v[j] = k < 245 ? rows[k / 7][2 * wo + k % 7] : 0.f;
    }
    out[e] = make_float4(v[0], v[1], v[2], v[3]);
  }
}

__global__ __launch_bounds__(256) void bn_partial2_kernel(const float* __restrict__ x, int64_t M, int C,
                                                          int64_t rows_per_block, double* __restrict__ part) {
  __shared__ double red[16][2][16][4];
  const int cq = threadIdx.x & 15, ry = threadIdx.x >> 4;
  const int c = blockIdx.x * 64 + cq * 4;
  const int64_t r0 = (int64_t)blockIdx.y * rows_per_block, r1 = min(M, r0 + rows_per_block);
  double s1[4] = {0.0, 0.0, 0.0, 0.0}, s2[4] = {0.0, 0.0, 0.0, 0.0};
  if (c < C) {
    const float4 sh4 = *reinterpret_cast<const float4*>(x + c);
    const double sh[4] = {(double)sh4.x, (double)sh4.y, (double)sh4.z, (double)sh4.w};
    for (int64_t r = r0 + ry; r < r1; r += 64) {
      float4 v4[4];
#pragma unroll
      for (int u = 0; u < 4; ++u)
        v4[u] = *reinterpret_cast<const float4*>(x + (r + 16 * u < r1 ? (r + 16 * u) * C : 0) + c);
#pragma unroll
      for (int u = 0; u < 4; ++u) {
        const float v[4] = {v4[u].x, v4[u].y, v4[u].z, v4[u].w};
#pragma unroll
        for (int j = 0; j < 4; ++j) {
          const double a = (double)v[j] - sh[j];
          s1[j] += a;
          s2[j] += a * a;
        }
      }
    }
  }
#pragma unroll
  for (int j = 0; j < 4; ++j) { red[ry][0][cq][j] = s1[j]; red[ry][1][cq][j] = s2[j]; }
  __syncthreads();
  if (ry < 2 && c < C) {
    double* out = part + ((int64_t)blockIdx.y * 2 + ry) * C + c;
#pragma unroll
    for (int j = 0; j < 4; ++j) {
      double t = red[0][ry][cq][j];
#pragma unroll
      for (int k = 1; k < 16; ++k) t += red[k][ry][cq][j];
      out[j] = t;
    }
  }
}

__global__ __launch_bounds__(1024) void bn_finalize2_kernel(const double* __restrict__ part, int nparts, int C, int64_t M,
                                                            const float* __restrict__ x, float eps, float momentum,
                                                            float* __restrict__ mean, float* __restrict__ var,
                                                            float* __restrict__ rstd, float* __restrict__ running_mean,
                                                            float* __restrict__ running_var, int64_t* __restrict__ nbt) {
  __shared__ double red[16][2][64];
  const int cx = threadIdx.x & 63, g = threadIdx.x >> 6;
  const int c = blockIdx.x * 64 + cx;
  double a = 0.0, b = 0.0;
  if (c < C) {
    int p = g;
    for (; p + 48 < nparts; p += 64) {
      const double a0 = part[((int64_t)p * 2 + 0) * C + c], a1 = part[((int64_t)(p + 16) * 2 + 0) * C + c];
      const double a2 = part[((int64_t)(p + 32) * 2 + 0) * C + c], a3 = part[((int64_t)(p + 48) * 2 + 0) * C + c];
      const double b0 = part[((int64_t)p * 2 + 1) * C + c], b1 = part[((int64_t)(p + 16) * 2 + 1) * C + c];
      const double b2 = part[((int64_t)(p + 32) * 2 + 1) * C + c], b3 = part[((int64_t)(p + 48) * 2 + 1) * C + c];
      a += a0; a += a1; a += a2; a += a3;
      b += b0; b += b1; b += b2; b += b3;
    }
    for (; p < nparts; p += 16) {
      a += part[((int64_t)p * 2 + 0) * C + c];
      b += part[((int64_t)p * 2 + 1) * C + c];
    }
  }
  red[g][0][cx] = a;
  red[g][1][cx] = b;
  __syncthreads();
  if (g != 0 || c >= C) return;
  a = b = 0.0;
#pragma unroll
  for (int q = 0; q < 16; ++q) { a += red[q][0][cx]; b += red[q][1][cx]; }
  const double d = a / (double)M;
  const double v = fmax(b / (double)M - d * d, 0.0);
// ... 189 lines not shown
  float acc[2][2][4];
  maxpool_block_grad(dy, idx, n, a, b, c4, Ho, Wo, C4, acc);
#pragma unroll
  for (int ph = 0; ph < 2; ++ph)
#pragma unroll
    for (int pw = 0; pw < 2; ++pw) {
      const int h = 2 * a + ph, w = 2 * b + pw;
      if (h < H && w < W)
        reinterpret_cast<float4*>(dx)[((n * H + h) * W + w) * C4 + c4] =
            make_float4(acc[ph][pw][0], acc[ph][pw][1], acc[ph][pw][2], acc[ph][pw][3]);
    }
}

__global__ __launch_bounds__(256) void bn_pool_bwd_reduce_kernel(const float* __restrict__ dpool, const uint8_t* __restrict__ idx,
                                                                 const float* __restrict__ x, const float* __restrict__ mean,
                                                                 const float* __restrict__ rstd, const float* __restrict__ gamma,
                                                                 const float* __restrict__ beta, int64_t nblocks, int H, int W,
                                                                 int Ho, int Wo, int C, int64_t blocks_per_wg, int act,
                                                                 float* __restrict__ part) {
  __shared__ float4 red[16][2][16];
  const int cq = threadIdx.x & 15, ry = threadIdx.x >> 4;
  const int c = blockIdx.x * 64 + cq * 4;
  const int C4 = C >> 2, H2 = (H + 1) >> 1, W2 = (W + 1) >> 1;
  const int64_t r0 = (int64_t)blockIdx.y * blocks_per_wg, r1 = min(nblocks, r0 + blocks_per_wg);
  float sb[4] = {0.f, 0.f, 0.f, 0.f}, sg[4] = {0.f, 0.f, 0.f, 0.f};
  if (c < C) {
    const float4 mu4 = *reinterpret_cast<const float4*>(mean + c), rs4 = *reinterpret_cast<const float4*>(rstd + c);
    const float4 g4 = *reinterpret_cast<const float4*>(gamma + c), b4 = *reinterpret_cast<const float4*>(beta + c);
    const float mu[4] = {mu4.x, mu4.y, mu4.z, mu4.w}, rs[4] = {rs4.x, rs4.y, rs4.z, rs4.w};
    const float g[4] = {g4.x, g4.y, g4.z, g4.w}, bt[4] = {b4.x, b4.y, b4.z, b4.w};
    for (int64_t r = r0 + ry; r < r1; r += 16) {
      const int b = (int)(r % W2), a = (int)((r / W2) % H2);
      const int64_t n = r / ((int64_t)W2 * H2);
      float acc[2][2][4];
      maxpool_block_grad(dpool, idx, n, a, b, c >> 2, Ho, Wo, C4, acc);
#pragma unroll
      for (int ph = 0; ph < 2; ++ph)
#pragma unroll
        for (int pw = 0; pw < 2; ++pw) {
          const int h = 2 * a + ph, w = 2 * b + pw;
          if (h >= H || w >= W) continue;
          const float4 xv4 = *reinterpret_cast<const float4*>(x + ((n * H + h) * W + w) * C + c);
          const float xv[4] = {xv4.x, xv4.y, xv4.z, xv4.w};
#pragma unroll
          for (int j = 0; j < 4; ++j) {
            const float xh = (xv[j] - mu[j]) * rs[j];
            const float d = acc[ph][pw][j] * act_bwd(act, xh * g[j] + bt[j]);
            sb[j] += d;
            sg[j] += d * xh;
          }
        }
    }
  }
  red[ry][0][cq] = make_float4(sb[0], sb[1], sb[2], sb[3]);
  red[ry][1][cq] = make_float4(sg[0], sg[1], sg[2], sg[3]);
  __syncthreads();
  if (ry < 2 && c < C) {
    float4 t = red[0][ry][cq];
#pragma unroll
    for (int k = 1; k < 16; ++k) { const float4 u = red[k][ry][cq]; t.x += u.x; t.y += u.y; t.z += u.z; t.w += u.w; }
    *reinterpret_cast<float4*>(part + ((int64_t)blockIdx.y * 2 + ry) * C + c) = t;
  }
}

__global__ void bn_pool_bwd_apply_kernel(const float* __restrict__ dpool, const uint8_t* __restrict__ idx,
                                         const float* __restrict__ x, const float* __restrict__ mean, const float* __restrict__ rstd,
                                         const float* __restrict__ gamma, const float* __restrict__ beta,
                                         const float* __restrict__ dgamma, const float* __restrict__ dbeta, float* __restrict__ dx,
                                         int H, int W, int Ho, int Wo, int C, int act, float invM, int64_t total4) {
  const int64_t i = (int64_t)blockIdx.x * blockDim.x + threadIdx.x;
  if (i >= total4) return;
  const int C4 = C >> 2, H2 = (H + 1) >> 1, W2 = (W + 1) >> 1;
  const int c4 = (int)(i % C4);
  int64_t r = i / C4;
  const int b = (int)(r % W2), a = (int)((r / W2) % H2);
  const int64_t n = r / ((int64_t)W2 * H2);
  float acc[2][2][4];
  maxpool_block_grad(dpool, idx, n, a, b, c4, Ho, Wo, C4, acc);
  const float4 mu4 = reinterpret_cast<const float4*>(mean)[c4], rs4 = reinterpret_cast<const float4*>(rstd)[c4];
  const float4 g4 = reinterpret_cast<const float4*>(gamma)[c4], b4 = reinterpret_cast<const float4*>(beta)[c4];
  const float4 dg4 = reinterpret_cast<const float4*>(dgamma)[c4], db4 = reinterpret_cast<const float4*>(dbeta)[c4];
  const float mu[4] = {mu4.x, mu4.y, mu4.z, mu4.w}, rs[4] = {rs4.x, rs4.y, rs4.z, rs4.w};
  const float g[4] = {g4.x, g4.y, g4.z, g4.w}, bt[4] = {b4.x, b4.y, b4.z, b4.w};
  const float dg[4] = {dg4.x, dg4.y, dg4.z, dg4.w}, db[4] = {db4.x, db4.y, db4.z, db4.w};
#pragma unroll
  for (int ph = 0; ph < 2; ++ph)
#pragma unroll
    for (int pw = 0; pw < 2; ++pw) {
      const int h = 2 * a + ph, w = 2 * b + pw;
      if (h >= H || w >= W) continue;
      const int64_t o = ((n * H + h) * W + w) * C4 + c4;
      const float4 xv4 = reinterpret_cast<const float4*>(x)[o];
      const float xv[4] = {xv4.x, xv4.y, xv4.z, xv4.w};
      float out[4];
#pragma unroll
      for (int j = 0; j < 4; ++j) {
        const float d = acc[ph][pw][j] * act_bwd(act, (xv[j] - mu[j]) * rs[j] * g[j] + bt[j]);
        out[j] = g[j] * rs[j] * (d - db[j] * invM - (xv[j] - mu[j]) * rs[j] * dg[j] * invM);
      }
      reinterpret_cast<float4*>(dx)[o] = make_float4(out[0], out[1], out[2], out[3]);
    }
}

__global__ void avgpool_fwd_kernel(const float* __restrict__ x, float* __restrict__ y, int P, int C, int64_t total) {
  const int64_t i = (int64_t)blockIdx.x * blockDim.x + threadIdx.x;
  if (i >= total) return;
  const int c = (int)(i % C);
  const int64_t n = i / C;
  float s = 0.f;
  for (int p = 0; p < P; ++p) s += x[(n * P + p) * C + c];
  y[i] = s / (float)P;
}
__global__ void avgpool_bwd_kernel(const float* __restrict__ dy, float* __restrict__ dx, int P, int C, int64_t total) {
  const int64_t i = (int64_t)blockIdx.x * blockDim.x + threadIdx.x;
  if (i >= total) return;
  const int c = (int)(i % C);
  const int64_t n = i / ((int64_t)C * P);
  dx[i] = dy[n * C + c] / (float)P;
}
__global__ void avgpool_bwd_vec_kernel(const float* __restrict__ dy, float* __restrict__ dx, int P, int C4, int64_t total4) {
  const int64_t i = (int64_t)blockIdx.x * blockDim.x + threadIdx.x;
  if (i >= total4) return;
  const int c4 = (int)(i % C4);
  const int64_t n = i / C4;
  float4 v = reinterpret_cast<const float4*>(dy)[i];
  v = make_float4(v.x / (float)P, v.y / (float)P, v.z / (float)P, v.w / (float)P);
  float4* o = reinterpret_cast<float4*>(dx) + n * P * C4 + c4;
  for (int p = 0; p < P; ++p) o[(int64_t)p * C4] = v;
}

__global__ void rsqrt_eps_kernel(const float* __restrict__ v, float eps, float* __restrict__ out, int64_t n) {
  const int64_t i = (int64_t)blockIdx.x * blockDim.x + threadIdx.x;
  if (i < n) out[i] = 1.f / sqrtf(v[i] + eps);
}

__global__ void copy2d_kernel(const float* __restrict__ src, int64_t lds, float* __restrict__ dst, int64_t ldd, int64_t N,
                              int64_t total) {
  const int64_t i = (int64_t)blockIdx.x * blockDim.x + threadIdx.x;
  if (i >= total) return;
  const int64_t m = i / N, n = i % N;
  dst[m * ldd + n] = src[m * lds + n];
}

__global__ void conv_wflip_kernel(const float* __restrict__ w2d, float* __restrict__ wflip, int Cout, int Cin) {
  const int64_t i = (int64_t)blockIdx.x * blockDim.x + threadIdx.x;
  const int64_t total = (int64_t)Cout * Cin * 9;
  if (i >= total) return;
  const int co = (int)(i % Cout);
  const int tap = (int)((i / Cout) % 9);
  const int ci = (int)(i / ((int64_t)Cout * 9));
  wflip[i] = w2d[(int64_t)co * 9 * Cin + (int64_t)(8 - tap) * Cin + ci];
}

__global__ void fill_kernel(float* __restrict__ p, float v, int64_t n) {
  const int64_t i = (int64_t)blockIdx.x * blockDim.x + threadIdx.x;
  if (i < n) p[i] = v;
}

static inline int bn_chunks(int64_t M) { return (int)std::min<int64_t>(std::max<int64_t>(1, M / 256), 1024); }

}

using namespace tavsr;

static inline dim3 grid1d(int64_t n) { return dim3((unsigned)((n + 255) / 256)); }

extern "C" int tavsr_im2col2d(const float* x, float* col, int64_t N, int32_t H, int32_t W, int32_t C, int32_t KH, int32_t KW,
                              int32_t stride, int32_t pad, tavsr_stream_t stream) {
  TAVSR_REQUIRE(x && col, TAVSR_EINVAL, "im2col2d: null pointer");
  TAVSR_REQUIRE(C % 4 == 0 && KH >= 1 && KW >= 1 && stride >= 1 && pad >= 0, TAVSR_EUNSUPPORTED, "im2col2d: C %% 4 == 0 required");
  const int Ho = (H + 2 * pad - KH) / stride + 1, Wo = (W + 2 * pad - KW) / stride + 1;
  const int64_t total4 = N * Ho * Wo * KH * KW * (C / 4);
  if (total4 <= 0) return TAVSR_OK;
  hipLaunchKernelGGL(im2col2d_kernel, grid1d(total4), dim3(256), 0, (hipStream_t)stream, x, col, H, W, Ho, Wo, C / 4, KH, KW,
                     stride, pad, total4);
  TAVSR_LAUNCH_CHECK();
  return TAVSR_OK;
}

extern "C" int tavsr_col2im2d(const float* dcol, float* dx, int64_t N, int32_t H, int32_t W, int32_t C, int32_t KH, int32_t KW,
                              int32_t stride, int32_t pad, const float* extra, tavsr_stream_t stream) {
  TAVSR_REQUIRE(dcol && dx, TAVSR_EINVAL, "col2im2d: null pointer");
  TAVSR_REQUIRE(C % 4 == 0 && KH >= 1 && KW >= 1 && stride >= 1 && pad >= 0, TAVSR_EUNSUPPORTED, "col2im2d: C %% 4 == 0 required");
  const int Ho = (H + 2 * pad - KH) / stride + 1, Wo = (W + 2 * pad - KW) / stride + 1;
  const int64_t total4 = N * H * W * (C / 4);
  if (total4 <= 0) return TAVSR_OK;
  hipLaunchKernelGGL(col2im2d_kernel, grid1d(total4), dim3(256), 0, (hipStream_t)stream, dcol, dx, H, W, Ho, Wo, C / 4, KH, KW,
                     stride, pad, total4, extra);
  TAVSR_LAUNCH_CHECK();
  return TAVSR_OK;
}

extern "C" int tavsr_im2col_stem(const float* x, float* col, int32_t B, int32_t T, int32_t H, int32_t W, tavsr_stream_t stream) {
  TAVSR_REQUIRE(x && col, TAVSR_EINVAL, "im2col_stem: null pointer");
  const int Ho = (H + 6 - 7) / 2 + 1, Wo = (W + 6 - 7) / 2 + 1;
  if ((int64_t)B * T * Ho * Wo <= 0) return TAVSR_OK;
  TAVSR_REQUIRE((int64_t)B * T * Ho < (1ll << 31) && W + 3 <= kStemLd && 2 * (Wo - 1) + 7 <= kStemLd, TAVSR_EUNSUPPORTED,
                "im2col_stem: frames up to %d pixels wide, fewer than 2^31 output rows (decode/eval goes through in slices)",
                kStemLd - 3);
  hipLaunchKernelGGL(im2col_stem_kernel, dim3((unsigned)((int64_t)B * T * Ho)), dim3(256), 0, (hipStream_t)stream, x, col, T, H, W,
                     Ho, Wo);
  TAVSR_LAUNCH_CHECK();
  return TAVSR_OK;
}

extern "C" int64_t tavsr_bn_ws(int64_t M, int32_t C) { return (int64_t)bn_chunks(M) * 4 * C; }

extern "C" int tavsr_bn_stats(const float* x, int64_t M, int32_t C, float eps, float momentum, float* mean, float* var,
                              float* rstd, float* running_mean, float* running_var, int64_t* num_batches_tracked, float* ws,
                              tavsr_stream_t stream) {
  TAVSR_REQUIRE(x && mean && var && rstd && ws, TAVSR_EINVAL, "bn_stats: null pointer");
  TAVSR_REQUIRE(M > 0 && C > 0, TAVSR_EINVAL, "bn_stats: empty input");
  TAVSR_REQUIRE(C % 4 == 0 && ((uintptr_t)x & 15) == 0 && ((uintptr_t)ws & 7) == 0, TAVSR_EUNSUPPORTED,
                "bn_stats: C %% 4 == 0, 16-byte aligned rows and an 8-byte aligned workspace required");
  hipStream_t s = (hipStream_t)stream;
  const int chunks = bn_chunks(M);
  const int64_t rpb = (M + chunks - 1) / chunks;
  const dim3 g(cdiv(C, 64), chunks);
  double* part = reinterpret_cast<double*>(ws);
  hipLaunchKernelGGL(bn_partial2_kernel, g, dim3(256), 0, s, x, M, C, rpb, part);
  hipLaunchKernelGGL(bn_finalize2_kernel, dim3(cdiv(C, 64)), dim3(1024), 0, s, (const double*)part, chunks, C, M, x, eps, momentum, mean, var, rstd,
                     running_mean, running_var, num_batches_tracked);
  TAVSR_LAUNCH_CHECK();
  return TAVSR_OK;
}

extern "C" int tavsr_bn_apply_fwd(const float* x, const float* mean, const float* rstd, const float* gamma, const float* beta,
                                  const float* res, float* y, int64_t M, int32_t C, int32_t act, tavsr_stream_t stream) {
  TAVSR_REQUIRE(x && mean && rstd && gamma && beta && y, TAVSR_EINVAL, "bn_apply_fwd: null pointer");
  TAVSR_REQUIRE(C % 4 == 0, TAVSR_EUNSUPPORTED, "bn_apply_fwd: C %% 4 == 0 required");
  const int64_t total4 = M * (C / 4);
  if (total4 <= 0) return TAVSR_OK;
  hipLaunchKernelGGL(bn_apply_fwd_kernel, grid1d(total4), dim3(256), 0, (hipStream_t)stream, x, mean, rstd, gamma, beta, res, y,
                     C / 4, act, total4);
  TAVSR_LAUNCH_CHECK();
  return TAVSR_OK;
}

extern "C" int tavsr_bn_bwd(const float* dy, const float* x, const float* mean, const float* rstd, const float* gamma,
                            const float* beta, const float* res, float* dz, float* dx, float* dgamma, float* dbeta, int64_t M,
                            int32_t C, int32_t act, float* ws, tavsr_stream_t stream) {
  TAVSR_REQUIRE(dy && x && mean && rstd && gamma && beta && dx && dgamma && dbeta && ws, TAVSR_EINVAL, "bn_bwd: null pointer");
  TAVSR_REQUIRE(dz || !res, TAVSR_EINVAL, "bn_bwd: dz (the gradient of res) is needed when there is a residual input");
  TAVSR_REQUIRE(C % 4 == 0, TAVSR_EUNSUPPORTED, "bn_bwd: C %% 4 == 0 required");
  if (M <= 0) return TAVSR_OK;
  hipStream_t s = (hipStream_t)stream;
  const int chunks = bn_chunks(M);
  const int64_t rpb = (M + chunks - 1) / chunks;
  hipLaunchKernelGGL(bn_bwd_reduce_kernel, dim3(cdiv(C, 64), chunks), dim3(256), 0, s, dy, x, mean, rstd, gamma, beta, res, dz, M,
                     C, rpb, act, ws);
  TAVSR_LAUNCH_CHECK();
  int rc = tavsr_sum_partials2(ws, chunks, (int64_t)2 * C, dbeta, C, dgamma, C, 0, stream);
  if (rc) return rc;
  const int64_t total4 = M * (C / 4);
  hipLaunchKernelGGL(bn_bwd_apply_kernel, grid1d(total4), dim3(256), 0, s, dz, x, mean, rstd, gamma, dgamma, dbeta, dx, C / 4,
                     1.f / (float)M, total4, dz ? nullptr : dy, beta, act);
  TAVSR_LAUNCH_CHECK();
  return TAVSR_OK;
}

extern "C" int tavsr_bn_bwd_pooled(const float* dpool, const uint8_t* idx, const float* x, const float* mean, const float* rstd,
                                   const float* gamma, const float* beta, float* dx, float* dgamma, float* dbeta, int64_t N,
                                   int32_t H, int32_t W, int32_t C, int32_t act, float* ws, tavsr_stream_t stream) {
  TAVSR_REQUIRE(dpool && idx && x && mean && rstd && gamma && beta && dx && dgamma && dbeta && ws, TAVSR_EINVAL,
                "bn_bwd_pooled: null pointer");
  TAVSR_REQUIRE(C % 4 == 0 && ((uintptr_t)idx & 3) == 0 && (((uintptr_t)dpool | (uintptr_t)x | (uintptr_t)dx) & 15) == 0,
                TAVSR_EUNSUPPORTED, "bn_bwd_pooled: C %% 4 == 0 and aligned tensors required");
  if (N <= 0 || H <= 0 || W <= 0) return TAVSR_OK;
  hipStream_t s = (hipStream_t)stream;
  const int Ho = (H + 2 - 3) / 2 + 1, Wo = (W + 2 - 3) / 2 + 1;
  const int64_t M = N * H * W, nblocks = N * ((H + 1) / 2) * ((W + 1) / 2);
  const int chunks = bn_chunks(M);
  const int64_t bpw = (nblocks + chunks - 1) / chunks;
  hipLaunchKernelGGL(bn_pool_bwd_reduce_kernel, dim3(cdiv(C, 64), chunks), dim3(256), 0, s, dpool, idx, x, mean, rstd, gamma, beta,
                     nblocks, H, W, Ho, Wo, C, bpw, act, ws);
  TAVSR_LAUNCH_CHECK();
  int rc = tavsr_sum_partials2(ws, chunks, (int64_t)2 * C, dbeta, C, dgamma, C, 0, stream);
  if (rc) return rc;
  const int64_t total4 = nblocks * (C / 4);
  hipLaunchKernelGGL(bn_pool_bwd_apply_kernel, grid1d(total4), dim3(256), 0, s, dpool, idx, x, mean, rstd, gamma, beta, dgamma, dbeta,
                     dx, H, W, Ho, Wo, C, act, 1.f / (float)M, total4);
  TAVSR_LAUNCH_CHECK();
  return TAVSR_OK;
}

extern "C" int tavsr_maxpool3x3s2_fwd(const float* x, float* y, uint8_t* idx, int64_t N, int32_t H, int32_t W, int32_t C,
                                      tavsr_stream_t stream) {
  TAVSR_REQUIRE(x && y && idx, TAVSR_EINVAL, "maxpool_fwd: null pointer");
  const int Ho = (H + 2 - 3) / 2 + 1, Wo = (W + 2 - 3) / 2 + 1;
  TAVSR_REQUIRE(C % 4 == 0 && (((uintptr_t)x | (uintptr_t)y) & 15) == 0 && ((uintptr_t)idx & 3) == 0, TAVSR_EUNSUPPORTED,
                "maxpool_fwd: C %% 4 == 0 and aligned tensors required");
  const int64_t total = N * Ho * Wo * (C / 4);
  if (total <= 0) return TAVSR_OK;
  hipLaunchKernelGGL(maxpool3x3s2_fwd_kernel, grid1d(total), dim3(256), 0, (hipStream_t)stream, x, y, idx, H, W, Ho, Wo, C, total,
                     (const float*)nullptr, (const float*)nullptr, (const float*)nullptr, (const float*)nullptr, 0);
  TAVSR_LAUNCH_CHECK();
  return TAVSR_OK;
}

extern "C" int tavsr_bn_act_maxpool3x3s2_fwd(const float* x, const float* mean, const float* rstd, const float* gamma,
                                             const float* beta, int32_t act, float* y, uint8_t* idx, int64_t N, int32_t H,
                                             int32_t W, int32_t C, tavsr_stream_t stream) {
  TAVSR_REQUIRE(x && mean && rstd && gamma && beta && y && idx, TAVSR_EINVAL, "bn_act_maxpool_fwd: null pointer");
  const int Ho = (H + 2 - 3) / 2 + 1, Wo = (W + 2 - 3) / 2 + 1;
  TAVSR_REQUIRE(C % 4 == 0 && (((uintptr_t)x | (uintptr_t)y | (uintptr_t)mean | (uintptr_t)rstd | (uintptr_t)gamma | (uintptr_t)beta) & 15) == 0 &&
                    ((uintptr_t)idx & 3) == 0, TAVSR_EUNSUPPORTED, "bn_act_maxpool_fwd: C %% 4 == 0 and aligned tensors required");
  const int64_t total = N * Ho * Wo * (C / 4);
  if (total <= 0) return TAVSR_OK;
  hipLaunchKernelGGL(maxpool3x3s2_fwd_kernel, grid1d(total), dim3(256), 0, (hipStream_t)stream, x, y, idx, H, W, Ho, Wo, C, total,
                     mean, rstd, gamma, beta, act);
  TAVSR_LAUNCH_CHECK();
  return TAVSR_OK;
}

extern "C" int tavsr_maxpool3x3s2_bwd(const float* dy, const uint8_t* idx, float* dx, int64_t N, int32_t H, int32_t W, int32_t C,
                                      tavsr_stream_t stream) {
  TAVSR_REQUIRE(dy && idx && dx, TAVSR_EINVAL, "maxpool_bwd: null pointer");
  const int Ho = (H + 2 - 3) / 2 + 1, Wo = (W + 2 - 3) / 2 + 1;
  TAVSR_REQUIRE(C % 4 == 0 && (((uintptr_t)dy | (uintptr_t)dx) & 15) == 0 && ((uintptr_t)idx & 3) == 0, TAVSR_EUNSUPPORTED,
                "maxpool_bwd: C %% 4 == 0 and aligned tensors required");
  const int64_t total = N * ((H + 1) / 2) * ((W + 1) / 2) * (C / 4);
  if (total <= 0) return TAVSR_OK;
  hipLaunchKernelGGL(maxpool3x3s2_bwd_kernel, grid1d(total), dim3(256), 0, (hipStream_t)stream, dy, idx, dx, H, W, Ho, Wo, C, total);
  TAVSR_LAUNCH_CHECK();
  return TAVSR_OK;
}

extern "C" int tavsr_avgpool_fwd(const float* x, float* y, int64_t N, int32_t P, int32_t C, tavsr_stream_t stream) {
  TAVSR_REQUIRE(x && y, TAVSR_EINVAL, "avgpool_fwd: null pointer");
  const int64_t total = N * C;
  if (total <= 0) return TAVSR_OK;
  hipLaunchKernelGGL(avgpool_fwd_kernel, grid1d(total), dim3(256), 0, (hipStream_t)stream, x, y, P, C, total);
  TAVSR_LAUNCH_CHECK();
  return TAVSR_OK;
}

extern "C" int tavsr_avgpool_bwd(const float* dy, float* dx, int64_t N, int32_t P, int32_t C, tavsr_stream_t stream) {
  TAVSR_REQUIRE(dy && dx, TAVSR_EINVAL, "avgpool_bwd: null pointer");
  const int64_t total = N * P * C;
  if (total <= 0) return TAVSR_OK;
  if (C % 4 == 0 && (((uintptr_t)dy | (uintptr_t)dx) & 15) == 0)
    hipLaunchKernelGGL(avgpool_bwd_vec_kernel, grid1d(N * (C / 4)), dim3(256), 0, (hipStream_t)stream, dy, dx, P, C / 4, N * (C / 4));
  else
    hipLaunchKernelGGL(avgpool_bwd_kernel, grid1d(total), dim3(256), 0, (hipStream_t)stream, dy, dx, P, C, total);
  TAVSR_LAUNCH_CHECK();
  return TAVSR_OK;
}

extern "C" int tavsr_rsqrt_eps(const float* v, float eps, float* out, int64_t n, tavsr_stream_t stream) {
  TAVSR_REQUIRE((v && out) || n <= 0, TAVSR_EINVAL, "rsqrt_eps: null pointer");
  if (n <= 0) return TAVSR_OK;
  hipLaunchKernelGGL(rsqrt_eps_kernel, grid1d(n), dim3(256), 0, (hipStream_t)stream, v, eps, out, n);
  TAVSR_LAUNCH_CHECK();
  return TAVSR_OK;
}

extern "C" int tavsr_copy2d(const float* src, int64_t lds, float* dst, int64_t ldd, int64_t M, int64_t N, tavsr_stream_t stream) {
  TAVSR_REQUIRE((src && dst) || M * N <= 0, TAVSR_EINVAL, "copy2d: null pointer");
  if (M * N <= 0) return TAVSR_OK;
  hipLaunchKernelGGL(copy2d_kernel, grid1d(M * N), dim3(256), 0, (hipStream_t)stream, src, lds, dst, ldd, N, M * N);
  TAVSR_LAUNCH_CHECK();
  return TAVSR_OK;
}

extern "C" int tavsr_conv_wflip(const float* w2d, float* wflip, int32_t Cout, int32_t Cin, tavsr_stream_t stream) {
  TAVSR_REQUIRE(w2d && wflip && Cout > 0 && Cin > 0, TAVSR_EINVAL, "conv_wflip: bad arguments");
  hipLaunchKernelGGL(conv_wflip_kernel, grid1d((int64_t)Cout * Cin * 9), dim3(256), 0, (hipStream_t)stream, w2d, wflip, Cout, Cin);
  TAVSR_LAUNCH_CHECK();
  return TAVSR_OK;
}

extern "C" int tavsr_fill(float* p, float value, int64_t n, tavsr_stream_t stream) {
  TAVSR_REQUIRE(p || n <= 0, TAVSR_EINVAL, "fill: null pointer");
  if (n <= 0) return TAVSR_OK;
  hipLaunchKernelGGL(fill_kernel, grid1d(n), dim3(256), 0, (hipStream_t)stream, p, value, n);
  TAVSR_LAUNCH_CHECK();
  return TAVSR_OK;
}
```

tailored-avsr_amd/tavsr/functional_av.py:

```python
from __future__ import annotations

import os
from typing import List, Optional

import torch

from . import ops
from ._lib import guarded
from .functional import DESC_FIELD, _draw_tokens, _note_ctx, _side_queue, _workspace
from .layer_blocks import (EPS_ESPNET, FF_PARAMS, FFM_PARAMS, AttnBranch, AttnSaved, CgmlpBranch, CgmlpSaved, FFNSaved, _FFN, _drop_,
                           _drop_bwd)

BN_EPS, BN_MOMENTUM = 1e-5, 0.1


def frontend_param_names() -> List[str]:
    names = ["frontend3D.0.weight", "frontend3D.1.weight", "frontend3D.1.bias"]
    inpl = 64
    for li, planes in enumerate((64, 128, 256, 512), start=1):
        for bi in range(2):
            p = f"trunk.layer{li}.{bi}."
            names += [p + "conv1.weight", p + "bn1.weight", p + "bn1.bias", p + "conv2.weight", p + "bn2.weight", p + "bn2.bias"]
            if bi == 0 and (li > 1 or inpl != planes):
                names += [p + "downsample.0.weight", p + "downsample.1.weight", p + "downsample.1.bias"]
        inpl = planes
    return names


def _w2d(w):
    co, ci, kh, kw = w.shape
    return ops.transpose_inner(w.contiguous(), co, ci, kh * kw).view(co, kh * kw * ci)


def _w2d_grad(g, shape):
    co, ci, kh, kw = shape
    return ops.transpose_inner(g, co, kh * kw, ci).view(shape)


def _conv3x3_dw(dz, x, N, H, W, cin, stride=1, taps=9):
    if dz.shape[0] % 32 == 0 and cin % 64 == 0:
        return ops.conv3x3_dw(dz, x, H, W, stride, taps)
    k = 3 if taps == 9 else 1
    col, _, _ = ops.im2col2d(x, N, H, W, cin, k, k, stride, k // 2)
    return ops.linear_dw(dz, col)


def _plan_env(name, default):
    v = os.environ.get(name)
    if v is None:
        return default
    return None if v in ("", "0") else tuple(int(t) for t in v.split(","))


STEM_DW_PLAN = _plan_env("TAVSR_STEM_DW_PLAN", (3, 512))
STEM_POOL_FUSED = True


class _BN:

    @staticmethod
    def stats(z, prefix, bufs, training):
        rm, rv, nbt = bufs[prefix + "running_mean"], bufs[prefix + "running_var"], bufs[prefix + "num_batches_tracked"]
        if training:
            return ops.bn_stats(z, BN_EPS, BN_MOMENTUM, rm, rv, nbt)
        return rm, ops.rsqrt_eps(rv, BN_EPS)


def _bn_eval_bwd(dy, z, mean, rstd, gamma, beta, res, act):
    raise NotImplementedError("backward through eval-mode BatchNorm is not on the reference's path (validation is no_grad)")


_FRONT_WGRAD_BESIDE = os.environ.get("TAVSR_FRONT_WGRAD_BESIDE", "1") != "0"


class VisualFrontendFn(torch.autograd.Function):
    @staticmethod
    def forward(ctx, x, cfg, *P):
        names = cfg["names"]
        p = dict(zip(names, P))
        bufs, training = cfg["buffers"], cfg["training"]
        B, T, H, W = x.shape
        N = B * T
        x = x.contiguous()
        saved = {}
        xp = col0 = w0 = None
        if ops.stem_pad16_ok(x):
            xp = ops.stem_pad(x)
            w0 = ops.stem_weight_288(p["frontend3D.0.weight"])
            z0, H0, W0 = ops.stem_conv_fwd_pad16(xp, w0, B, T, H, W)
        else:
            w0 = ops.fill_(ops.empty(64, 256, like=x), 0.0)
            ops.copy2d(p["frontend3D.0.weight"].reshape(64, 245), w0[:, :245])
            if ops.stem_implicit_ok(x):
                z0, H0, W0 = ops.stem_conv_fwd(x, w0)
            else:
                col0, H0, W0 = ops.im2col_stem(x)
                z0 = ops.linear(col0, w0)
        m0, r0 = _BN.stats(z0, "frontend3D.1.", bufs, training)
        if STEM_POOL_FUSED:
            cur, idx0, Hc, Wc = ops.bn_act_maxpool3x3s2_fwd(z0, m0, r0, p["frontend3D.1.weight"], p["frontend3D.1.bias"], "swish",
                                                            N, H0, W0, 64)
        else:
            y0 = ops.bn_apply_fwd(z0, m0, r0, p["frontend3D.1.weight"], p["frontend3D.1.bias"], None, "swish")
            cur, idx0, Hc, Wc = ops.maxpool3x3s2_fwd(y0, N, H0, W0, 64)
            del y0
        saved["stem"] = (x if xp is None else xp, z0, m0, r0, idx0, H0, W0, w0, col0, xp is not None)
        blocks = []
        cin = 64
        for li, planes in enumerate((64, 128, 256, 512), start=1):
            for bi in range(2):
                pre = f"trunk.layer{li}.{bi}."
                stride = 2 if (li > 1 and bi == 0) else 1
                has_ds = (pre + "downsample.0.weight") in p
                Xin, Hin, Win = cur, Hc, Wc
                w1 = _w2d(p[pre + "conv1.weight"])
                Ho, Wo = (Hin - 1) // stride + 1, (Win - 1) // stride + 1
                z1 = ops.conv3x3_fwd(Xin, w1, Hin, Win, stride)
                m1, r1 = _BN.stats(z1, pre + "bn1.", bufs, training)
                y1 = ops.bn_apply_fwd(z1, m1, r1, p[pre + "bn1.weight"], p[pre + "bn1.bias"], None, "swish")
                w2 = _w2d(p[pre + "conv2.weight"])
                z2 = ops.conv3x3_fwd(y1, w2, Ho, Wo)
                m2, r2 = _BN.stats(z2, pre + "bn2.", bufs, training)
                ds = None
                if has_ds:
                    wd = _w2d(p[pre + "downsample.0.weight"])
                    zd = ops.conv3x3_fwd(Xin, wd, Hin, Win, stride, taps=1)
                    md, rd = _BN.stats(zd, pre + "downsample.1.", bufs, training)
                    res = ops.bn_apply_fwd(zd, md, rd, p[pre + "downsample.1.weight"], p[pre + "downsample.1.bias"], None, None)
                    ds = (zd, md, rd, wd)
                else:
                    res = Xin
                cur = ops.bn_apply_fwd(z2, m2, r2, p[pre + "bn2.weight"], p[pre + "bn2.bias"], res, "swish")
                blocks.append((pre, stride, cin, planes, Hin, Win, Ho, Wo, Xin, z1, m1, r1, w1, z2, m2, r2, w2, res, ds, y1))
                cin, Hc, Wc = planes, Ho, Wo
        feat = ops.avgpool_fwd(cur, N, Hc * Wc, cin)
        ctx.saved, ctx.blocks, ctx.p, ctx.names = saved, blocks, p, names
        ctx.dims = (B, T, N, Hc, Wc, cin)
        ctx.training = training
        return feat.view(B, T, cin)

    @staticmethod
    @guarded
    def backward(ctx, dfeat):
        if not ctx.training:
            _bn_eval_bwd(None, None, None, None, None, None, None, None)
        p = ctx.p
        B, T, N, Hc, Wc, cl = ctx.dims
        G = {}
        d = ops.avgpool_bwd(dfeat.contiguous().view(N, cl), N, Hc * Wc, cl)
        beside = _FRONT_WGRAD_BESIDE and ops.wgrad_may_go_beside(list(p.values()))

        def wgrad(name, fn):
            if beside:
                ops.wgrad_beside(lambda: G.__setitem__(name, fn()))
            else:
                G[name] = fn()

        def self_ds_bwd(ds, dres, pre, Xin, N, Hin, Win, cin, stride):
            zd, md, rd, wd = ds
            _, dzd, G[pre + "downsample.1.weight"], G[pre + "downsample.1.bias"] = ops.bn_bwd(
                dres, zd, md, rd, p[pre + "downsample.1.weight"], p[pre + "downsample.1.bias"], None, None, need_dz=False)
            wgrad(pre + "downsample.0.weight", lambda: _w2d_grad(_conv3x3_dw(dzd, Xin, N, Hin, Win, cin, stride, taps=1),
                                                                 p[pre + "downsample.0.weight"].shape))
            return ops.linear_dx(dzd, wd)

        for (pre, stride, cin, planes, Hin, Win, Ho, Wo, Xin, z1, m1, r1, w1, z2, m2, r2, w2, res, ds, y1) in reversed(ctx.blocks):
            dres, dz2, G[pre + "bn2.weight"], G[pre + "bn2.bias"] = ops.bn_bwd(
                d, z2, m2, r2, p[pre + "bn2.weight"], p[pre + "bn2.bias"], res, "swish")
            wgrad(pre + "conv2.weight", lambda: _w2d_grad(_conv3x3_dw(dz2, y1, N, Ho, Wo, planes), p[pre + "conv2.weight"].shape))
            dy1 = ops.conv3x3_dx(dz2, ops.conv_wflip(w2, planes, planes), Ho, Wo)
            _, dz1, G[pre + "bn1.weight"], G[pre + "bn1.bias"] = ops.bn_bwd(
                dy1, z1, m1, r1, p[pre + "bn1.weight"], p[pre + "bn1.bias"], None, "swish", need_dz=False)
            fused_ds = False
            if stride == 1:
                wgrad(pre + "conv1.weight", lambda: _w2d_grad(_conv3x3_dw(dz1, Xin, N, Hin, Win, cin), p[pre + "conv1.weight"].shape))
                dX = ops.conv3x3_dx(dz1, ops.conv_wflip(w1, planes, cin), Hin, Win, res=None if ds is not None else dres)
            else:
                wgrad(pre + "conv1.weight", lambda: _w2d_grad(_conv3x3_dw(dz1, Xin, N, Hin, Win, cin, stride), p[pre + "conv1.weight"].shape))
                dcol1 = ops.linear_dx(dz1, w1)
                dcold = None
                if ds is not None:
                    dcold = self_ds_bwd(ds, dres, pre, Xin, N, Hin, Win, cin, stride)
                dX = ops.col2im2d(dcol1, N, Hin, Win, cin, 3, 3, stride, 1, extra=dcold)
                del dcol1
                fused_ds = ds is not None
            if ds is not None and not fused_ds:
                dcold = self_ds_bwd(ds, dres, pre, Xin, N, Hin, Win, cin, stride)
                dXd = ops.col2im2d(dcold, N, Hin, Win, cin, 1, 1, stride, 0)
                d = ops.axpby(dX, dXd, 1.0, 1.0)
            elif stride == 1 or fused_ds:
                d = dX
            else:
                d = ops.axpby(dX, dres, 1.0, 1.0)
        x, z0, m0, r0, idx0, H0, W0, w0, col0, padded = ctx.saved["stem"]
        dz0, G["frontend3D.1.weight"], G["frontend3D.1.bias"] = ops.bn_bwd_pooled(
            d.contiguous(), idx0, z0, m0, r0, p["frontend3D.1.weight"], p["frontend3D.1.bias"], N, H0, W0, "swish")
        if padded:
            T_ = ctx.dims[1]
            gw0 = ops.stem_conv_dw_pad16(dz0, x, T_, 2 * H0, 2 * W0)
            G["frontend3D.0.weight"] = ops.stem_weight_grad_from_288(gw0, p["frontend3D.0.weight"].shape)
        else:
            if col0 is None:
                gw0 = ops.stem_conv_dw(dz0, x)
            else:
                gw0 = ops.linear_dw(dz0, col0, force=STEM_DW_PLAN)
            g0 = ops.empty(64, 245, like=gw0)
            ops.copy2d(gw0[:, :245], g0)
            G["frontend3D.0.weight"] = g0.view(p["frontend3D.0.weight"].shape)
        del col0
        ctx.saved = ctx.blocks = None
        return (None, None, *[G[n] for n in ctx.names])


class ScaleFn(torch.autograd.Function):

    @staticmethod
    def forward(ctx, x, s):
        ctx.s = s
        return ops.axpby(x.contiguous(), None, s, 0.0)

    @staticmethod
    @guarded
    def backward(ctx, dy):
        return ops.axpby(dy.contiguous(), None, ctx.s, 0.0), None


class PadTimeFn(torch.autograd.Function):

    @staticmethod
    def forward(ctx, x, p, value):
        B, T, D = x.shape
        x = x.contiguous()
        out = ops.fill_(ops.empty(B, T + p, D, like=x), float(value))
        ops.copy2d(x.view(B, T * D), out.view(B, (T + p) * D)[:, : T * D])
        ctx.dims = (B, T, D)
        return out

    @staticmethod
    @guarded
    def backward(ctx, dy):
        B, T, D = ctx.dims
        dy = dy.contiguous()
        dx = ops.empty(B, T * D, like=dy)
        ops.copy2d(dy.view(B, -1)[:, : T * D], dx)
        return dx.view(B, T, D), None, None


class AddRowFn(torch.autograd.Function):

    @staticmethod
    def forward(ctx, x, row):
        shp = x.shape
        x2 = x.contiguous().view(-1, shp[-1])
        y, _ = ops.add_head_bias(x2, row.contiguous(), row.contiguous())
        return y.view(shp)

    @staticmethod
    @guarded
    def backward(ctx, dy):
        d2 = dy.contiguous().view(-1, dy.shape[-1])
        return dy, ops.colsum(d2)


TS_SHARED = ("norm_ff_macaron.weight", "norm_ff_macaron.bias",
             "feed_forward_macaron.w_1.weight", "feed_forward_macaron.w_1.bias",
             "feed_forward_macaron.w_2.weight", "feed_forward_macaron.w_2.bias",
             "norm_ff.weight", "norm_ff.bias", "feed_forward.w_1.weight", "feed_forward.w_1.bias",
             "feed_forward.w_2.weight", "feed_forward.w_2.bias", "norm_final.weight", "norm_final.bias")
TS_ATTN = ("norm_mha.weight", "norm_mha.bias", "attn.linear_q.weight", "attn.linear_q.bias", "attn.linear_k.weight",
           "attn.linear_k.bias", "attn.linear_v.weight", "attn.linear_v.bias", "attn.linear_out.weight",
           "attn.linear_out.bias", "attn.linear_pos.weight", "attn.pos_bias_u", "attn.pos_bias_v")
TS_MLP = ("norm_cgmlp.weight", "norm_cgmlp.bias", "cgmlp.channel_proj1.0.weight", "cgmlp.channel_proj1.0.bias",
          "cgmlp.csgu.norm.weight", "cgmlp.csgu.norm.bias", "cgmlp.csgu.conv.weight", "cgmlp.csgu.conv.bias",
          "cgmlp.channel_proj2.weight", "cgmlp.channel_proj2.bias")


def tailored_stream_param_names(use_attn: bool):
    return TS_SHARED + (TS_ATTN if use_attn else TS_MLP)


def _ts_branch_fwd(p, cfg, x1, n, mean, rstd, pos_emb, lens, B, T, need):
    coeff, pd = cfg.get("coeff", 1.0), cfg.get("p", 0.0)
    if cfg["use_attn"]:
        cx, s = AttnBranch.fwd(n, p, pos_emb, lens, B, T, cfg["heads"], cfg.get("p_att", 0.0))
        x2, t_br = ops.linear_drop(cx, p["attn.linear_out.weight"], p["attn.linear_out.bias"], pd, alpha=coeff, res=x1)
        return x2, s._replace(mean=mean, rstd=rstd, t_br=t_br)
    w1c, cw = p["cgmlp.channel_proj1.0.weight"], p["cgmlp.csgu.conv.weight"]
    if ops.BLOCKS_C and ops.cgmlp_block_ok(n, w1c, cw) and x1.is_contiguous():
        x2, (g, z, gn, gmean, grstd, u, conv, t_u, t_br), _ = ops.cgmlp_fwd(
            n, w1c, p["cgmlp.channel_proj1.0.bias"], p["cgmlp.csgu.norm.weight"], p["cgmlp.csgu.norm.bias"], cw,
            p["cgmlp.csgu.conv.bias"], p["cgmlp.channel_proj2.weight"], p["cgmlp.channel_proj2.bias"], B, T, p=pd, p_out=pd, alpha=coeff,
            res=x1, save=need)
        return x2, CgmlpSaved(mean=mean, rstd=rstd, n=n, g=g, z=z, gn=gn, gmean=gmean, grstd=grstd, u=u, conv=conv, t_u=t_u, t_br=t_br)
    u, s = CgmlpBranch.fwd(n, p, B, T, pd, need)
    x2, t_br = ops.linear_drop(u, p["cgmlp.channel_proj2.weight"], p["cgmlp.channel_proj2.bias"], pd, alpha=coeff, res=x1)
    return x2, s._replace(mean=mean, rstd=rstd, t_br=t_br)


def _ts_branch_bwd(p, cfg, saved, dx2, x1, pos_emb, lens, B, T, grp, lng, G, dbr=None, out_drop=None):
    coeff = cfg.get("coeff", 1.0)
    dbr = _drop_bwd(dx2, saved.t_br) if dbr is None else dbr
    if cfg["use_attn"]:
        bn = "norm_mha"
        dn, _ = AttnBranch.bwd(dbr, saved, p, pos_emb, lens, B, T, cfg["heads"], grp, G, alpha=coeff)
    else:
        bn = "norm_cgmlp"
        dn = CgmlpBranch.bwd(dbr, saved, p, B, T, grp, G, alpha=coeff)
    dx1, G[bn + ".weight"], G[bn + ".bias"], *dxd = lng.bwd(dn, x1, saved.mean, saved.rstd, p[bn + ".weight"], dx_add=dx2, drop=out_drop)
    return (dx1, dxd[0]) if dxd else dx1


class TailoredStreamFn(torch.autograd.Function):
    @staticmethod
    def forward(ctx, x, pos_emb, lens, cfg, *P):
        names = tailored_stream_param_names(cfg["use_attn"])
        p = dict(zip(names, P))
        B, T, D = x.shape
        M = B * T
        act = cfg["ffn_act"]
        pd = cfg.get("p", 0.0)
        need = cfg.get("need_bwd", True)
        x2d = x.contiguous().view(M, D)
        sv = {}
        bn = "norm_mha" if cfg["use_attn"] else "norm_cgmlp"
        x1, sv["ffm"], (n,), mean, rstd = _FFN.fwd_ln(x2d, *[p[k] for k in FFM_PARAMS], act, 0.5, [(p[bn + ".weight"], p[bn + ".bias"])],
                                                      p=pd, save=need)
        x2, sv["br"] = _ts_branch_fwd(p, cfg, x1, n, mean, rstd, pos_emb, lens, B, T, need)
        x3, sv["ff"], (y,), fmean, frstd = _FFN.fwd_ln(x2, *[p[k] for k in FF_PARAMS], act, 0.5,
                                                       [(p["norm_final.weight"], p["norm_final.bias"])], p=pd, save=need)
# ... 270 lines not shown
```

tailored-avsr_amd/tavsr/ops/__init__.py:

```python
from __future__ import annotations

import os
from typing import Optional

PROFILE: Optional[GemmProfile] = None

WGRAD_BESIDE = os.environ.get("TAVSR_WGRAD_BESIDE", "1") != "0"
WGRAD_SLOT = int(os.environ.get("TAVSR_WGRAD_SLOT", "0"))

LN_BWD_DROP = True

ATTN_FUSED = True

FFN2 = True
FFN2_BWD = True
FFN2_BWD_LN = os.environ.get("TAVSR_FFN2_BWD_LN", "1") != "0"

LAYER_C = os.environ.get("TAVSR_LAYER_C", "1") != "0"
LAYER_C_EAGER_ONLY = os.environ.get("TAVSR_LAYER_C", "1") != "capture"
BLOCKS_C = os.environ.get("TAVSR_BLOCKS_C", "1") != "0"

CSGU_FUSED = True
CSGU_STATS_IN_GEMM = True
CGMLP_ACT_BWD_FUSED = True

MERGE_ROWS = True
MERGE_PROJ = os.environ.get("TAVSR_MERGE_PROJ", "1") == "1"
MERGE_ROWDOT = True

STEM_IMPLICIT = True
STEM_PAD16 = True

CONV_TAPSKIP = os.environ.get("TAVSR_CONV_TAPSKIP", "1") != "0"
CONV_TAPSKIP_MAXPOS = int(os.environ.get("TAVSR_CONV_TAPSKIP_MAXPOS", "121"))
CONV_TILEORDER = os.environ.get("TAVSR_CONV_TILEORDER", "1") != "0"
CONV_TAPSKIP_MAXPOS_DW = int(os.environ.get("TAVSR_CONV_TAPSKIP_MAXPOS_DW", "36"))
CONV_DW_UNEVEN = os.environ.get("TAVSR_CONV_DW_UNEVEN", "1") != "0"

CONV_TAPSKIP_STRIDE2 = os.environ.get("TAVSR_CONV_TAPSKIP_STRIDE2", "1") != "0"
CONV_TAPSKIP_STRIDE2_DW = os.environ.get("TAVSR_CONV_TAPSKIP_STRIDE2_DW", "0") != "0"
CONV_TAPSKIP_STRIDE2_MAXPOS = 36

CTC_ALIGN_CHUNK = 16

RESAMPLE_ROLLOFF, RESAMPLE_ZEROS, RESAMPLE_BETA = 0.9475937167399596, 64, 14.769656459379492

ROWLIN = True
ROWLIN_KSPLIT = 4
TREE_ROWS_MAX_KEYS = 1024
RNNT_SEARCH_KINDS = {"alsd": 0, "tsd": 1}
RNNT_SEARCH_LIMIT = ("1 <= beam <= 64, beam < vocabulary, at least one frame, u_max >= 0, 1 <= max_sym_exp <= 8, the trie of an "
                     "utterance within 2^30 words")

RNNT_WS_FLOATS = 1 << 24

from .base import *
from .rng import *
from .streams import *
from .data import *
from .blocks import *
from .matmul import *
from .norm import *
from .attention import *
from .vision import *
from .losses import *
from .search import *
from .rnnt import *
```

tailored-avsr_amd/tavsr/ops/vision.py:

```python
from __future__ import annotations

import torch

from .. import ops
from .._lib import ACT, check, lib, ptr, require_cuda, stream
from .base import empty
from .matmul import gemm

__all__ = ["conv1_fwd", "conv1_bwd", "im2col3x3s2", "col2im3x3s2_relu", "conv_out", "im2col2d", "col2im2d", "stem_implicit_ok",
           "stem_pad16_ok", "stem_pad", "stem_weight_288", "stem_weight_grad_from_288", "stem_conv_fwd_pad16", "stem_conv_dw_pad16",
           "stem_conv_fwd", "stem_conv_dw", "im2col_stem", "bn_stats", "rsqrt_eps", "bn_apply_fwd", "bn_bwd", "bn_bwd_pooled",
           "maxpool3x3s2_fwd", "bn_act_maxpool3x3s2_fwd", "maxpool3x3s2_bwd", "avgpool_fwd", "avgpool_bwd", "conv_wflip", "_tapskip",
           "_tapskip2", "_tapskip_any", "conv3x3_fwd", "conv3x3_dx", "conv3x3_dw"]


def conv1_fwd(x, w, bias):
    B, T, F = x.shape
    Cn = w.shape[0]
    To, Fo = (T - 3) // 2 + 1, (F - 3) // 2 + 1
    y = empty(B, To, Fo, Cn, like=x)
    require_cuda(x, w, bias)
    check(lib().tavsr_conv1_fwd(ptr(x), ptr(w), ptr(bias), ptr(y), B, T, F, Cn, stream()), "tavsr_conv1_fwd")
    return y


def conv1_bwd(dz, x, Cn):
    B, T, F = x.shape
    dw, db = empty(Cn, 9, like=x), empty(Cn, like=x)
    ws = empty(lib().tavsr_conv1_bwd_ws(B, T, F, Cn), like=x)
    check(lib().tavsr_conv1_bwd(ptr(dz), ptr(x), ptr(dw), ptr(db), 0, ptr(ws), B, T, F, Cn, stream()), "tavsr_conv1_bwd")
    return dw, db


def im2col3x3s2(y):
    B, Ti, Fi, Cn = y.shape
    To, Fo = (Ti - 3) // 2 + 1, (Fi - 3) // 2 + 1
    col = empty(B * To * Fo, 9 * Cn, like=y)
    check(lib().tavsr_im2col3x3s2(ptr(y), ptr(col), B, Ti, Fi, Cn, stream()), "tavsr_im2col3x3s2")
    return col, To, Fo


def col2im3x3s2_relu(dcol, yrelu):
    B, Ti, Fi, Cn = yrelu.shape
    dz = torch.empty_like(yrelu)
    check(lib().tavsr_col2im3x3s2_relu(ptr(dcol), ptr(yrelu), ptr(dz), B, Ti, Fi, Cn, stream()), "tavsr_col2im3x3s2_relu")
    return dz


def conv_out(n, k, s, p):
    return (n + 2 * p - k) // s + 1


def im2col2d(x, N, H, W, Cn, KH, KW, stride, pad):
    require_cuda(x)
    Ho, Wo = conv_out(H, KH, stride, pad), conv_out(W, KW, stride, pad)
    col = empty(N * Ho * Wo, KH * KW * Cn, like=x)
    check(lib().tavsr_im2col2d(ptr(x), ptr(col), N, H, W, Cn, KH, KW, stride, pad, stream()), "tavsr_im2col2d")
    return col, Ho, Wo


def col2im2d(dcol, N, H, W, Cn, KH, KW, stride, pad, extra=None):
    require_cuda(dcol, extra)
    assert extra is None or (extra.is_contiguous() and extra.shape == (dcol.shape[0], Cn))
    dx = empty(N * H * W, Cn, like=dcol)
    check(lib().tavsr_col2im2d(ptr(dcol), ptr(dx), N, H, W, Cn, KH, KW, stride, pad, ptr(extra), stream()), "tavsr_col2im2d")
    return dx


def stem_implicit_ok(x) -> bool:
    B, T, H, W = x.shape
    Ho, Wo = conv_out(H, 7, 2, 3), conv_out(W, 7, 2, 3)
    return (ops.STEM_IMPLICIT and H % 2 == 0 and W % 2 == 0 and W >= 8 and (B * T * Ho * Wo) % 32 == 0 and T < 1024 and H < 1000 and W < 1000
            and B * T * H * W < 2 ** 31 and x.data_ptr() % 16 == 0)


def stem_pad16_ok(x) -> bool:
    B, T, H, W = x.shape
    Ho, Wo = H // 2, W // 2
    return (ops.STEM_IMPLICIT and ops.STEM_PAD16 and H % 2 == 0 and W % 4 == 0 and (B * T * Ho * Wo) % 32 == 0
            and B * (T + 5) * (H + 6) * (W + 8) < 2 ** 31)


def stem_pad(x):
    return torch.nn.functional.pad(x, (3, 5, 3, 3, 2, 3)).contiguous()


def stem_weight_288(w):
    co = w.shape[0]
    return torch.nn.functional.pad(torch.nn.functional.pad(w.reshape(co, 35, 7), (0, 1)).reshape(co, 280), (0, 8)).contiguous()


def stem_weight_grad_from_288(g, shape):
    co = g.shape[0]
    return g[:, :280].reshape(co, 35, 8)[:, :, :7].reshape(shape).contiguous()


def stem_conv_fwd_pad16(xp, w288, B, T, H, W):
    Ho, Wo = H // 2, W // 2
    M = B * T * Ho * Wo
    z = empty(M, w288.shape[0], like=xp)
    gemm(M, w288.shape[0], 288, xp, 4, w288, 288, z, w288.shape[0], conv=(6, H + 6, W + 8, T + 5))
    return z, Ho, Wo


def stem_conv_dw_pad16(dz, xp, T, H, W):
    M, cout = dz.shape
    dw = empty(cout, 288, like=dz)
    gemm(cout, 288, M, dz, cout, xp, 4, dw, 288, a_kmajor=True, b_kmajor=True, conv=(7, H + 6, W + 8, T + 5))
    return dw


def stem_conv_fwd(x, w0p):
    B, T, H, W = x.shape
    Ho, Wo = conv_out(H, 7, 2, 3), conv_out(W, 7, 2, 3)
    M = B * T * Ho * Wo
    z = empty(M, w0p.shape[0], like=x)
    gemm(M, w0p.shape[0], 256, x, 4, w0p, 256, z, w0p.shape[0], conv=(4, H, W, T))
    return z, Ho, Wo


def stem_conv_dw(dz, x):
    B, T, H, W = x.shape
    M, cout = dz.shape
    dw = empty(cout, 256, like=dz)
    gemm(cout, 256, M, dz, cout, x, 4, dw, 256, a_kmajor=True, b_kmajor=True, conv=(5, H, W, T))
    return dw


def im2col_stem(x):
    B, T, H, W = x.shape
    require_cuda(x)
    Ho, Wo = conv_out(H, 7, 2, 3), conv_out(W, 7, 2, 3)
    col = empty(B * T * Ho * Wo, 256, like=x)
    check(lib().tavsr_im2col_stem(ptr(x), ptr(col), B, T, H, W, stream()), "tavsr_im2col_stem")
    return col, Ho, Wo


def bn_stats(x, eps, momentum, running_mean=None, running_var=None, nbt=None):
    M, Cn = x.shape
    require_cuda(x, running_mean, running_var, nbt)
    mean, var, rstd = empty(Cn, like=x), empty(Cn, like=x), empty(Cn, like=x)
    ws = empty(lib().tavsr_bn_ws(M, Cn), like=x)
    check(lib().tavsr_bn_stats(ptr(x), M, Cn, eps, momentum, ptr(mean), ptr(var), ptr(rstd), ptr(running_mean), ptr(running_var), ptr(nbt),
                               ptr(ws), stream()), "tavsr_bn_stats")
    return mean, rstd


def rsqrt_eps(v, eps):
    out = torch.empty_like(v)
    check(lib().tavsr_rsqrt_eps(ptr(v), eps, ptr(out), v.numel(), stream()), "tavsr_rsqrt_eps")
    return out


def bn_apply_fwd(x, mean, rstd, gamma, beta, res=None, act=None):
    M, Cn = x.shape
    require_cuda(x, mean, rstd, gamma, beta, res)
    y = torch.empty_like(x)
    check(lib().tavsr_bn_apply_fwd(ptr(x), ptr(mean), ptr(rstd), ptr(gamma), ptr(beta), ptr(res), ptr(y), M, Cn, ACT[act], stream()),
          "tavsr_bn_apply_fwd")
    return y


def bn_bwd(dy, x, mean, rstd, gamma, beta, res=None, act=None, need_dz=True):
    M, Cn = x.shape
    require_cuda(dy, x, mean, rstd, gamma, beta, res)
    assert need_dz or res is None
    dz, dx = (torch.empty_like(x) if need_dz else None), torch.empty_like(x)
    dg, db = empty(Cn, like=x), empty(Cn, like=x)
    ws = empty(lib().tavsr_bn_ws(M, Cn), like=x)
    check(lib().tavsr_bn_bwd(ptr(dy), ptr(x), ptr(mean), ptr(rstd), ptr(gamma), ptr(beta), ptr(res), ptr(dz), ptr(dx), ptr(dg), ptr(db), M,
                             Cn, ACT[act], ptr(ws), stream()), "tavsr_bn_bwd")
    return dz, dx, dg, db


def bn_bwd_pooled(dpool, idx, x, mean, rstd, gamma, beta, N, H, W, act=None):
    M, Cn = x.shape
    require_cuda(dpool, idx, x, mean, rstd, gamma, beta)
    assert M == N * H * W and dpool.is_contiguous() and idx.dtype == torch.uint8 and idx.is_contiguous()
    dx = torch.empty_like(x)
    dg, db = empty(Cn, like=x), empty(Cn, like=x)
    ws = empty(lib().tavsr_bn_ws(M, Cn), like=x)
    check(lib().tavsr_bn_bwd_pooled(ptr(dpool), ptr(idx), ptr(x), ptr(mean), ptr(rstd), ptr(gamma), ptr(beta), ptr(dx), ptr(dg), ptr(db), N,
                                    H, W, Cn, ACT[act], ptr(ws), stream()), "tavsr_bn_bwd_pooled")
    return dx, dg, db


def maxpool3x3s2_fwd(x, N, H, W, Cn):
    Ho, Wo = conv_out(H, 3, 2, 1), conv_out(W, 3, 2, 1)
    y = empty(N * Ho * Wo, Cn, like=x)
    idx = torch.empty((N * Ho * Wo, Cn), dtype=torch.uint8, device=x.device)
    check(lib().tavsr_maxpool3x3s2_fwd(ptr(x), ptr(y), ptr(idx), N, H, W, Cn, stream()), "tavsr_maxpool3x3s2_fwd")
    return y, idx, Ho, Wo


def bn_act_maxpool3x3s2_fwd(z, mean, rstd, gamma, beta, act, N, H, W, Cn):
    Ho, Wo = conv_out(H, 3, 2, 1), conv_out(W, 3, 2, 1)
    require_cuda(z, mean, rstd, gamma, beta)
    y = empty(N * Ho * Wo, Cn, like=z)
    idx = torch.empty((N * Ho * Wo, Cn), dtype=torch.uint8, device=z.device)
    check(lib().tavsr_bn_act_maxpool3x3s2_fwd(ptr(z), ptr(mean), ptr(rstd), ptr(gamma), ptr(beta), ACT[act], ptr(y), ptr(idx), N, H, W, Cn,
                                              stream()), "tavsr_bn_act_maxpool3x3s2_fwd")
    return y, idx, Ho, Wo


def maxpool3x3s2_bwd(dy, idx, N, H, W, Cn):
    dx = empty(N * H * W, Cn, like=dy)
    check(lib().tavsr_maxpool3x3s2_bwd(ptr(dy), ptr(idx), ptr(dx), N, H, W, Cn, stream()), "tavsr_maxpool3x3s2_bwd")
    return dx


def avgpool_fwd(x, N, P, Cn):
    y = empty(N, Cn, like=x)
    check(lib().tavsr_avgpool_fwd(ptr(x), ptr(y), N, P, Cn, stream()), "tavsr_avgpool_fwd")
    return y


def avgpool_bwd(dy, N, P, Cn):
    dx = empty(N * P, Cn, like=dy)
    check(lib().tavsr_avgpool_bwd(ptr(dy), ptr(dx), N, P, Cn, stream()), "tavsr_avgpool_bwd")
    return dx


def conv_wflip(w2d, cout, cin):
    require_cuda(w2d)
    out = empty(cin, 9 * cout, like=w2d)
    check(lib().tavsr_conv_wflip(ptr(w2d), ptr(out), cout, cin, stream()), "tavsr_conv_wflip")
    return out


def _tapskip_bits():
    return 1 | (0 if ops.CONV_TILEORDER else 2) | (0 if ops.CONV_DW_UNEVEN else 4)


def _tapskip(H, W, stride=1, taps=9, pad0=False, dw=False):
    on = ops.CONV_TAPSKIP and stride == 1 and taps == 9 and not pad0 and H * W <= (ops.CONV_TAPSKIP_MAXPOS_DW if dw else ops.CONV_TAPSKIP_MAXPOS)
    return _tapskip_bits() if on else 0


def _tapskip2(H, W, dw=False):
    on = ops.CONV_TAPSKIP and (ops.CONV_TAPSKIP_STRIDE2_DW if dw else ops.CONV_TAPSKIP_STRIDE2)
    return (_tapskip_bits() | 8) if on and ((H - 1) // 2 + 1) * ((W - 1) // 2 + 1) <= ops.CONV_TAPSKIP_STRIDE2_MAXPOS else 0


def _tapskip_any(H, W, stride, taps, pad0, dw=False):
    return _tapskip2(H, W, dw) if stride == 2 and taps == 9 and not pad0 else _tapskip(H, W, stride, taps, pad0, dw)


def conv3x3_fwd(x, w2d, H, W, stride=1, taps=9, pad0=False, bias=None, act=None):
    M, cin = x.shape
    cout = w2d.shape[0]
    if pad0:
        assert taps == 9
        Ho, Wo = (H - 3) // stride + 1, (W - 3) // stride + 1
    else:
        Ho, Wo = (H - 1) // stride + 1, (W - 1) // stride + 1
    Mo = M // (H * W) * Ho * Wo
    z = empty(Mo, cout, like=x)
    gemm(Mo, cout, taps * cin, x, cin, w2d, taps * cin, z, cout, conv=(1, H, W, cin, stride, 90 if pad0 else taps, _tapskip_any(H, W, stride, taps, pad0)),
         bias=bias, act=act)
    return z


def conv3x3_dx(dz, wflip, H, W, res=None):
    M, cout = dz.shape
    cin = wflip.shape[0]
    dx = empty(M, cin, like=dz)
    gemm(M, cin, 9 * cout, dz, cout, wflip, 9 * cout, dx, cin, conv=(1, H, W, cout, 0, 0, _tapskip(H, W)), R=res, ldr=0 if res is None else cin)
    return dx


def conv3x3_dw(dz, x, H, W, stride=1, taps=9, pad0=False, bias_grad=False, force=None):
    M, cout = dz.shape
    cin = x.shape[1]
    dw = empty(cout, taps * cin, like=dz)
    gb = empty(cout, like=dz) if bias_grad else None
    gemm(cout, taps * cin, M, dz, cout, x, cin, dw, taps * cin, a_kmajor=True, b_kmajor=True,
         conv=(2, H, W, cin, stride, 90 if pad0 else taps, _tapskip_any(H, W, stride, taps, pad0, dw=True)), a_rowsum=gb, force=force)
    return (dw, gb) if bias_grad else dw
```

Measured before the change: 412.1.

## Run f32 conv GEMMs on bf16 MFMA with three-way operand splitting

Adds an X6 path for implicit-GEMM 3x3 convolutions (forward and data-grad). Both operands are split into high/mid/low bf16 parts, and the product is rebuilt from six bf16 MFMA products to emulate f32 accuracy. Weights are pre-split into planes by a new wsplit kernel, and the activation tile is split in registers per k-block. The aim is to use the higher bf16 matrix throughput instead of the f32 path, at the cost of extra split arithmetic, a larger B stage in LDS, a weight-split launch per call, and slightly different numerics.

```diff
diff --git a/include/tavsr.h b/include/tavsr.h
--- a/include/tavsr.h
+++ b/include/tavsr.h
@@ -490,6 +490,7 @@
 int tavsr_avgpool_bwd(const float* dy, float* dx, int64_t N, int32_t P, int32_t C, tavsr_stream_t stream);
 int tavsr_fill(float* p, float value, int64_t n, tavsr_stream_t stream);
 int tavsr_conv_wflip(const float* w2d, float* wflip, int32_t Cout, int32_t Cin, tavsr_stream_t stream);
+int tavsr_conv_wsplit(const float* w, int64_t ld, float* out, int32_t N, int32_t K, tavsr_stream_t stream);
 int tavsr_copy2d(const float* src, int64_t lds, float* dst, int64_t ldd, int64_t M, int64_t N, tavsr_stream_t stream);
 
 int tavsr_stft_frames(const float* wav, const float* window, float* frames, int32_t B, int64_t N, int32_t T, int32_t n_fft,
diff --git a/tailored-avsr_amd/csrc/gemm_conv.hip b/tailored-avsr_amd/csrc/gemm_conv.hip
--- a/tailored-avsr_amd/csrc/gemm_conv.hip
+++ b/tailored-avsr_amd/csrc/gemm_conv.hip
@@ -111,11 +111,15 @@
 struct SourceFor<1, false, BM, BN, NT, false, BKM> {
   using type = PairSource<ConvRowsA<BM, NT>, PlainOperand<BN, BKM, NT, true>, BM>;
 };
-
-template <int BM, int BN, int NT, bool BKM>
+template <int BM, int BN, int NT>
+struct SourceFor<1, false, BM, BN, NT, false, false, true> {
+  using type = PairSource<ConvRowsA<BM, NT>, PlaneOperand<BN, NT>, BM>;
+};
+
+template <int BM, int BN, int NT, bool BKM, bool X6 = false>
 struct PosMajorRowsSource : SourceDefaults {
   using R = ImageRows<BM, NT>;
-  using LB = GLoader<BN, BKM, NT>;
+  using LB = std::conditional_t<X6, PlaneLoader<BN, NT>, GLoader<BN, BKM, NT>>;
   static constexpr int kDma = R::L::NR + LB::NR;
   static constexpr bool kPosMajorRows = true;
   const TileCtx& c;
@@ -124,12 +128,13 @@
   int tap, cb, nk;
   bool c9;
   R rows;
-  int64_t offB[LB::NR];
+  std::conditional_t<X6, int, int64_t> offB[LB::NR];
   __device__ __forceinline__ explicit PosMajorRowsSource(const TileCtx& c_) : c(c_) {
     const tavsr_gemm_desc& d = c.d;
     const ConvGeom g(d);
     c9 = g.c9;
-    LB::offsets(d.ldb, c.n0, d.N, c.tid, offB);
+    if constexpr (X6) LB::offsets(d.K, c.n0, d.N, c.tid, offB);
+    else LB::offsets(d.ldb, c.n0, d.N, c.tid, offB);
     pm.H = g.Ho; pm.W = g.Wo;
     pm.st = g.cs; pm.HI = d.conv_H; pm.WI = d.conv_W;
     pm.n = d.M / (g.Ho * g.Wo);
@@ -180,12 +185,17 @@
     cb = wrap ? 0 : cb + 1;
     tap = !wrap ? tap : up ? __builtin_ctz(up) : 9;
     rows.issue(c, c9, kk, ktap, stage);
-    LB::issue(c.B + (BKM ? (int64_t)kk * d.ldb : kk), offB, stage + BM * kBK, c.wave);
+    if constexpr (X6) LB::issue(x6_planes(d) + kk / 2, offB, stage + BM * kBK, c.wave);
+    else LB::issue(c.B + (BKM ? (int64_t)kk * d.ldb : kk), offB, stage + BM * kBK, c.wave);
   }
 };
 template <int BM, int BN, int NT, bool BKM>
 struct SourceFor<1, true, BM, BN, NT, false, BKM> {
   using type = PosMajorRowsSource<BM, BN, NT, BKM>;
+};
+template <int BM, int BN, int NT>
+struct SourceFor<1, true, BM, BN, NT, false, false, true> {
+  using type = PosMajorRowsSource<BM, BN, NT, false, true>;
 };
 
 template <int BN, int NT>
@@ -572,7 +582,7 @@
 constexpr int kPmStride2MaxPos = 36;
 static bool conv_pm(const tavsr_gemm_desc& d) {
   const bool stride_ok = d.conv_stride <= 1 || (d.conv_stride == 2 && (d.conv_posmajor & 8) && conv_ho(d) * conv_wo(d) <= kPmStride2MaxPos);
-  return d.conv_posmajor && (d.conv_mode == 1 || d.conv_mode == 2) && stride_ok && (d.conv_taps == 0 || d.conv_taps == 9) &&
+  return (d.conv_posmajor & ~kConvX6) && (d.conv_mode == 1 || d.conv_mode == 2) && stride_ok && (d.conv_taps == 0 || d.conv_taps == 9) &&
          (d.conv_mode == 2 || !d.a_rowsum);
 }
 
@@ -619,7 +629,7 @@
   last_o = o;
 }
 
-template <int BM, int BN, int MINW, bool AK, bool BKM, int CONV, bool PM>
+template <int BM, int BN, int MINW, bool AK, bool BKM, int CONV, bool PM, bool X6 = false, int WM = 2, int WN = 2, int S = 2>
 static int launch_conv_tile(const tavsr_gemm_desc& d, const Plan& p, hipStream_t s) {
   const int zmap = (CONV == 2 || CONV == 5 || CONV == 7) && p.nsplit >= 8 && p.nsplit % 8 == 0;
   const bool two = PM && CONV == 2;
@@ -628,23 +638,36 @@
   if constexpr (PM && CONV == 1) {
     GemmArgsOrd ao{a, {}};
     tile_order_build(d, BM, p.nsplit, ao.ord);
-    hipLaunchKernelGGL((gemm_glds_kernel<BM, BN, 2, 2, 2, MINW, AK, BKM, 1, CONV, true>), grid, dim3(256), 0, s, ao);
+    hipLaunchKernelGGL((gemm_glds_kernel<BM, BN, WM, WN, S, MINW, AK, BKM, 1, CONV, true, X6>), grid, dim3(WM * WN * 64), 0, s, ao);
   } else {
-    hipLaunchKernelGGL((gemm_glds_kernel<BM, BN, 2, 2, 2, MINW, AK, BKM, 1, CONV, PM>), grid, dim3(256), 0, s, a);
+    hipLaunchKernelGGL((gemm_glds_kernel<BM, BN, WM, WN, S, MINW, AK, BKM, 1, CONV, PM, X6>), grid, dim3(WM * WN * 64), 0, s, a);
   }
   TAVSR_LAUNCH_CHECK();
   return launch_epilogue(a, s);
 }
 
-template <int BM, int BN, int MINW, bool AK, bool BKM, int CONV>
+template <int BM, int BN, int MINW, bool AK, bool BKM, int CONV, bool X6 = false, int WM = 2, int WN = 2, int S = 2>
 static int launch_conv_pm(const tavsr_gemm_desc& d, const Plan& p, hipStream_t s) {
-  return conv_pm(d) ? launch_conv_tile<BM, BN, MINW, AK, BKM, CONV, true>(d, p, s) : launch_conv_tile<BM, BN, MINW, AK, BKM, CONV, false>(d, p, s);
+  return conv_pm(d) ? launch_conv_tile<BM, BN, MINW, AK, BKM, CONV, true, X6, WM, WN, S>(d, p, s)
+                    : launch_conv_tile<BM, BN, MINW, AK, BKM, CONV, false, X6, WM, WN, S>(d, p, s);
+}
+
+static bool conv_x6(const tavsr_gemm_desc& d, const Plan& p) {
+  return (d.conv_posmajor & kConvX6) && d.conv_mode == 1 && !d.a_kmajor && !d.b_kmajor && d.ldb == d.K &&
+         (d.conv_taps == 0 || d.conv_taps == 9 || (d.conv_taps == 1 && d.K >= 256)) && aligned16(d.B) && (int64_t)d.N * d.K * 6 < (1ll << 31);
 }
 
 int launch_conv(const tavsr_gemm_desc& d, const Plan& p, hipStream_t s) {
   switch (d.conv_mode) {
     case 1:
       if (d.b_kmajor) return launch_conv_pm<64, 64, 5, false, true, 1>(d, p, s);
+      if (conv_x6(d, p)) {
+        const bool big = p.nsplit == 1 && (int64_t)cdiv(d.M, 128) * cdiv(d.N, d.N % 128 == 0 ? 128 : 64) >= 512;
+        if (big && d.N % 128 == 0) return launch_conv_pm<128, 128, 2, false, false, 1, true>(d, p, s);
+        if (big) return launch_conv_pm<128, 64, 2, false, false, 1, true, 4, 1>(d, p, s);
+        if (p.nsplit == 1 && d.N % 128 == 0) return launch_conv_pm<64, 128, 2, false, false, 1, true>(d, p, s);
+        return launch_conv_pm<64, 64, 4, false, false, 1, true>(d, p, s);
+      }
       if (p.nsplit == 1 && d.N % 128 == 0) return launch_conv_pm<64, 128, 3, false, false, 1>(d, p, s);
       return launch_conv_pm<64, 64, 5, false, false, 1>(d, p, s);
     case 2:
diff --git a/tailored-avsr_amd/csrc/gemm_glds.h b/tailored-avsr_amd/csrc/gemm_glds.h
--- a/tailored-avsr_amd/csrc/gemm_glds.h
+++ b/tailored-avsr_amd/csrc/gemm_glds.h
@@ -379,6 +379,57 @@
   }
 }
 
+typedef __bf16 bf16x2 __attribute__((ext_vector_type(2)));
+typedef __bf16 bf16x8 __attribute__((ext_vector_type(8)));
+typedef float f32x2 __attribute__((ext_vector_type(2)));
+constexpr int kX6RowFloats = 48;
+
+__device__ __forceinline__ uint32_t pk_bf16(float a, float b) {
+  f32x2 v = {a, b};
+  return __builtin_bit_cast(uint32_t, __builtin_convertvector(v, bf16x2));
+}
+__device__ __forceinline__ void split_pair(float a, float b, uint32_t& h, uint32_t& m, uint32_t& l) {
+  h = pk_bf16(a, b);
+  a -= __uint_as_float(h << 16);
+  b -= __uint_as_float(h & 0xffff0000u);
+  m = pk_bf16(a, b);
+  a -= __uint_as_float(m << 16);
+  b -= __uint_as_float(m & 0xffff0000u);
+  l = pk_bf16(a, b);
+}
+__device__ __forceinline__ void split_frag(const float (&f)[8], uint4& h, uint4& m, uint4& l) {
+  split_pair(f[0], f[1], h.x, m.x, l.x);
+  split_pair(f[2], f[3], h.y, m.y, l.y);
+  split_pair(f[4], f[5], h.z, m.z, l.z);
+  split_pair(f[6], f[7], h.w, m.w, l.w);
+}
+__device__ __forceinline__ f32x16 mfma_bf16(const uint4& a, const uint4& b, const f32x16& c) {
+  return __builtin_amdgcn_mfma_f32_32x32x16_bf16(__builtin_bit_cast(bf16x8, a), __builtin_bit_cast(bf16x8, b), c, 0, 0, 0);
+}
+
+template <int ROWS, int NT>
+struct PlaneLoader {
+  static constexpr int NR = ROWS * 12 / NT;
+  static_assert(ROWS * 12 % NT == 0 && (ROWS * 4) % 64 == 0, "a wave instruction stays inside one plane");
+  __device__ static __forceinline__ void offsets(int K, int row0, int nrows, int tid, int (&off)[NR]) {
+#pragma unroll
+    for (int i = 0; i < NR; ++i) {
+      const int q = i * NT + tid, plane = q / (ROWS * 4), r = q % (ROWS * 4);
+      const int row = r >> 2, cl = (r & 3) ^ ((row >> 2) & 3);
+      off[i] = (plane * nrows + min(row0 + row, nrows - 1)) * (K / 2) + cl * 4;
+    }
+  }
+  __device__ static __forceinline__ void issue(const float* __restrict__ gk, const int (&off)[NR], float* __restrict__ img, int wave) {
+#pragma unroll
+    for (int i = 0; i < NR; ++i)
+      __builtin_amdgcn_global_load_lds((glb_float*)(gk + off[i]), (lds_float*)(img + (i * NT + wave * 64) * 4), 16, 0, 0);
+  }
+};
+template <int ROWS>
+__device__ __forceinline__ uint4 read_plane(const float* __restrict__ s, int p, int row, int b, int lk) {
+  return *reinterpret_cast<const uint4*>(s + ((p * ROWS + row) * 4 + ((2 * b + lk) ^ ((row >> 2) & 3))) * 4);
+}
+
 template <int N>
 __device__ __forceinline__ void wait_vmcnt() {
   asm volatile("s_waitcnt vmcnt(%0)" ::"n"(N) : "memory");
@@ -440,6 +491,22 @@
   __device__ __forceinline__ void issue(int kt, float* img) { L::issue(gk + kt * kstep, off, img, c.wave); }
 };
 
+constexpr int kConvX6 = 16;
+__device__ __forceinline__ const float* x6_planes(const tavsr_gemm_desc& d) { return d.B + (int64_t)d.N * d.K; }
+template <int ROWS, int NT>
+struct PlaneOperand {
+  using L = PlaneLoader<ROWS, NT>;
+  static constexpr int kDma = L::NR;
+  const TileCtx& c;
+  int off[L::NR];
+  const float* gk;
+  __device__ __forceinline__ explicit PlaneOperand(const TileCtx& c_) : c(c_) {
+    L::offsets(c.d.K, c.n0, c.d.N, c.tid, off);
+    gk = x6_planes(c.d) + c.kbeg / 2;
+  }
+  __device__ __forceinline__ void issue(int kt, float* img) { L::issue(gk + kt * (kBK / 2), off, img, c.wave); }
+};
+
 template <class HA, class HB, int BM>
 struct PairSource : SourceDefaults {
   static constexpr int kDma = HA::kDma + HB::kDma;
@@ -454,23 +521,24 @@
   }
 };
 
-template <int CONV, bool PM, int BM, int BN, int NT, bool AK, bool BKM>
+template <int CONV, bool PM, int BM, int BN, int NT, bool AK, bool BKM, bool X6 = false>
 struct SourceFor;
 template <int BM, int BN, int NT, bool AK, bool BKM>
 struct SourceFor<0, false, BM, BN, NT, AK, BKM> {
   using type = PairSource<PlainOperand<BM, AK, NT, false>, PlainOperand<BN, BKM, NT, true>, BM>;
 };
 
-template <int BM, int BN, int WM, int WN, int S, bool AK, bool BKM, int KW = 1, int CONV = 0, bool PM = false>
+template <int BM, int BN, int WM, int WN, int S, bool AK, bool BKM, int KW = 1, int CONV = 0, bool PM = false, bool X6 = false>
 __device__ __forceinline__ void glds_tile(const tavsr_gemm_desc& d, int kchunk, int nsplit, int tiles_n, int bid, bool vec_epi,
                                           int zidx, int n_big = 0, int kunit = 0) {
   constexpr int BK = kBK, NG = BK / 8;
   static_assert(NG % KW == 0, "k-groups must divide over the wave sets");
   static_assert(!PM || KW == 1, "position-major order: one wave set");
+  static_assert(!X6 || (CONV == 1 && !AK && !BKM && KW == 1), "split operands: CONV 1, both operands k-contiguous, one wave set");
   constexpr int NT = WM * WN * KW * 64;
   constexpr int TM = BM / WM / 32, TN = BN / WN / 32;
-  using Src = typename SourceFor<CONV, PM, BM, BN, NT, AK, BKM>::type;
-  constexpr int ASZ = BM * BK, STAGE = (BM + BN) * BK;
+  using Src = typename SourceFor<CONV, PM, BM, BN, NT, AK, BKM, X6>::type;
+  constexpr int ASZ = BM * BK, STAGE = BM * BK + BN * (X6 ? kX6RowFloats : BK);
   constexpr int G = Src::kDma;
   static_assert((S - 2) * G <= 63, "vmcnt field");
   __shared__ __attribute__((aligned(1024))) float smem[S * STAGE];
@@ -518,6 +586,48 @@
   auto compute = [&](int st) {
     const float* a_s = smem + st * STAGE;
     const float* b_s = a_s + ASZ;
+    if constexpr (X6) {
+      float af[2][TM][8];
+      uint4 bq[2][TN][3];
+      auto read_block = [&](int b, float (&fa)[TM][8], uint4 (&qb)[TN][3]) {
+#pragma unroll
+        for (int i = 0; i < TM; ++i) {
+          float lo[4], hi[4];
+          read_frag_g<BM, false>(a_s, arow + i * 32, 2 * b, lk, lo);
+          read_frag_g<BM, false>(a_s, arow + i * 32, 2 * b + 1, lk, hi);
+#pragma unroll
+          for (int e = 0; e < 4; ++e) { fa[i][e] = lo[e]; fa[i][4 + e] = hi[e]; }
+        }
+#pragma unroll
+        for (int j = 0; j < TN; ++j)
+#pragma unroll
+          for (int p = 0; p < 3; ++p) qb[j][p] = read_plane<BN>(b_s, p, brow + j * 32, b, lk);
+      };
+      read_block(0, af[0], bq[0]);
+#pragma unroll
+      for (int b = 0; b < BK / 16; ++b) {
+        const int c = b & 1;
+        if (b + 1 < BK / 16) read_block(b + 1, af[c ^ 1], bq[c ^ 1]);
+        GEMM_SB();
+        uint4 ah[TM], am[TM], al[TM];
+#pragma unroll
+        for (int i = 0; i < TM; ++i) split_frag(af[c][i], ah[i], am[i], al[i]);
+#pragma unroll
+        for (int pr = 0; pr < 6; ++pr) {
+          constexpr int PA[6] = {0, 2, 1, 0, 1, 0}, PB[6] = {2, 0, 1, 1, 0, 0};
+#pragma unroll
+          for (int i = 0; i < TM; ++i)
+#pragma unroll
+            for (int j = 0; j < TN; ++j)
+              acc[i][j] = mfma_bf16(PA[pr] == 0 ? ah[i] : PA[pr] == 1 ? am[i] : al[i], bq[c][j][PB[pr]], acc[i][j]);
+        }
+#pragma unroll
+        for (int i = 0; i < TM; ++i)
+          asum[i] += ((af[c][i][0] + af[c][i][1]) + (af[c][i][2] + af[c][i][3])) + ((af[c][i][4] + af[c][i][5]) + (af[c][i][6] + af[c][i][7]));
+        GEMM_SB();
+      }
+      return;
+    }
     float af[2][TM][4], bf[2][TN][4];
 #pragma unroll
     for (int i = 0; i < TM; ++i) read_frag_g<BM, AK>(a_s, arow + i * 32, kw, lk, af[0][i]);
@@ -653,12 +763,12 @@
   }
 };
 
-template <int BM, int BN, int WM, int WN, int S, int MINW, bool AK, bool BKM, int KW = 1, int CONV = 0, bool PM = false>
+template <int BM, int BN, int WM, int WN, int S, int MINW, bool AK, bool BKM, int KW = 1, int CONV = 0, bool PM = false, bool X6 = false>
 __global__ __launch_bounds__(WM* WN * KW * 64, MINW)
 void gemm_glds_kernel(const std::conditional_t<PM && CONV == 1, GemmArgsOrd, GemmArgs> xargs) {
   int bid, zidx;
   const GemmArgs& args = TileMap<CONV, PM>::map(xargs, bid, zidx);
-  glds_tile<BM, BN, WM, WN, S, AK, BKM, KW, CONV, PM>(args.d, args.kchunk, args.nsplit, args.tiles_n, bid, args.vec_epi != 0, zidx,
+  glds_tile<BM, BN, WM, WN, S, AK, BKM, KW, CONV, PM, X6>(args.d, args.kchunk, args.nsplit, args.tiles_n, bid, args.vec_epi != 0, zidx,
                                                       args.n_big, args.kunit);
 }
 
diff --git a/tailored-avsr_amd/csrc/vision.hip b/tailored-avsr_amd/csrc/vision.hip
--- a/tailored-avsr_amd/csrc/vision.hip
+++ b/tailored-avsr_amd/csrc/vision.hip
@@ -3,6 +3,7 @@
 #include <algorithm>
 
 #include "common.h"
+#include "gemm_glds.h"
 
 namespace tavsr {
 
@@ -498,6 +499,26 @@
   wflip[i] = w2d[(int64_t)co * 9 * Cin + (int64_t)(8 - tap) * Cin + ci];
 }
 
+__global__ void conv_wsplit_kernel(const float* __restrict__ w, int64_t ld, float* __restrict__ out, int N, int K) {
+  const int64_t i = (int64_t)blockIdx.x * blockDim.x + threadIdx.x;
+  const int cpr = K / 8;
+  if (i >= (int64_t)N * cpr) return;
+  const int n = (int)(i / cpr), ch = (int)(i % cpr), b = ch >> 1, lk = ch & 1;
+  const float* src = w + (int64_t)n * ld + 16 * b + 4 * lk;
+  const float4 lo = *reinterpret_cast<const float4*>(src), hi = *reinterpret_cast<const float4*>(src + 8);
+  const float f[8] = {lo.x, lo.y, lo.z, lo.w, hi.x, hi.y, hi.z, hi.w};
+  float* cp = out + (int64_t)n * K + 16 * b + 4 * lk;
+  *reinterpret_cast<float4*>(cp) = lo;
+  *reinterpret_cast<float4*>(cp + 8) = hi;
+  uint4* planes = reinterpret_cast<uint4*>(out + (int64_t)N * K);
+  uint4 h, m, l;
+  split_frag(f, h, m, l);
+  const int64_t plane = (int64_t)N * cpr;
+  planes[i] = h;
+  planes[plane + i] = m;
+  planes[2 * plane + i] = l;
+}
+
 __global__ void fill_kernel(float* __restrict__ p, float v, int64_t n) {
   const int64_t i = (int64_t)blockIdx.x * blockDim.x + threadIdx.x;
   if (i < n) p[i] = v;
@@ -716,6 +737,15 @@
   return TAVSR_OK;
 }
 
+extern "C" int tavsr_conv_wsplit(const float* w, int64_t ld, float* out, int32_t N, int32_t K, tavsr_stream_t stream) {
+  TAVSR_REQUIRE(w && out && N > 0 && K > 0, TAVSR_EINVAL, "conv_wsplit: bad arguments");
+  TAVSR_REQUIRE(K % 16 == 0 && ld % 4 == 0 && ld >= K && (((uintptr_t)w | (uintptr_t)out) & 15) == 0, TAVSR_EUNSUPPORTED,
+                "conv_wsplit: K %% 16 == 0 and 16-byte aligned rows");
+  hipLaunchKernelGGL(conv_wsplit_kernel, grid1d((int64_t)N * (K / 8)), dim3(256), 0, (hipStream_t)stream, w, ld, out, N, K);
+  TAVSR_LAUNCH_CHECK();
+  return TAVSR_OK;
+}
+
 extern "C" int tavsr_fill(float* p, float value, int64_t n, tavsr_stream_t stream) {
   TAVSR_REQUIRE(p || n <= 0, TAVSR_EINVAL, "fill: null pointer");
   if (n <= 0) return TAVSR_OK;
diff --git a/tailored-avsr_amd/tavsr/functional_av.py b/tailored-avsr_amd/tavsr/functional_av.py
--- a/tailored-avsr_amd/tavsr/functional_av.py
+++ b/tailored-avsr_amd/tavsr/functional_av.py
@@ -30,6 +30,10 @@
 def _w2d(w):
     co, ci, kh, kw = w.shape
     return ops.transpose_inner(w.contiguous(), co, ci, kh * kw).view(co, kh * kw * ci)
+
+
+def _planes(w, taps=9):
+    return ops.conv_wsplit(w) if ops.x6_takes(w, taps) else None
 
 
 def _w2d_grad(g, shape):
@@ -115,16 +119,16 @@
                 Xin, Hin, Win = cur, Hc, Wc
                 w1 = _w2d(p[pre + "conv1.weight"])
                 Ho, Wo = (Hin - 1) // stride + 1, (Win - 1) // stride + 1
-                z1 = ops.conv3x3_fwd(Xin, w1, Hin, Win, stride)
+                z1 = ops.conv3x3_fwd(Xin, w1, Hin, Win, stride, planes=_planes(w1))
                 m1, r1 = _BN.stats(z1, pre + "bn1.", bufs, training)
                 y1 = ops.bn_apply_fwd(z1, m1, r1, p[pre + "bn1.weight"], p[pre + "bn1.bias"], None, "swish")
                 w2 = _w2d(p[pre + "conv2.weight"])
-                z2 = ops.conv3x3_fwd(y1, w2, Ho, Wo)
+                z2 = ops.conv3x3_fwd(y1, w2, Ho, Wo, planes=_planes(w2))
                 m2, r2 = _BN.stats(z2, pre + "bn2.", bufs, training)
                 ds = None
                 if has_ds:
                     wd = _w2d(p[pre + "downsample.0.weight"])
-                    zd = ops.conv3x3_fwd(Xin, wd, Hin, Win, stride, taps=1)
+                    zd = ops.conv3x3_fwd(Xin, wd, Hin, Win, stride, taps=1, planes=_planes(wd, 1))
                     md, rd = _BN.stats(zd, pre + "downsample.1.", bufs, training)
                     res = ops.bn_apply_fwd(zd, md, rd, p[pre + "downsample.1.weight"], p[pre + "downsample.1.bias"], None, None)
                     ds = (zd, md, rd, wd)
@@ -168,13 +172,15 @@
             dres, dz2, G[pre + "bn2.weight"], G[pre + "bn2.bias"] = ops.bn_bwd(
                 d, z2, m2, r2, p[pre + "bn2.weight"], p[pre + "bn2.bias"], res, "swish")
             wgrad(pre + "conv2.weight", lambda: _w2d_grad(_conv3x3_dw(dz2, y1, N, Ho, Wo, planes), p[pre + "conv2.weight"].shape))
-            dy1 = ops.conv3x3_dx(dz2, ops.conv_wflip(w2, planes, planes), Ho, Wo)
+            wf2 = ops.conv_wflip(w2, planes, planes)
+            dy1 = ops.conv3x3_dx(dz2, wf2, Ho, Wo, planes=_planes(wf2))
             _, dz1, G[pre + "bn1.weight"], G[pre + "bn1.bias"] = ops.bn_bwd(
                 dy1, z1, m1, r1, p[pre + "bn1.weight"], p[pre + "bn1.bias"], None, "swish", need_dz=False)
             fused_ds = False
             if stride == 1:
                 wgrad(pre + "conv1.weight", lambda: _w2d_grad(_conv3x3_dw(dz1, Xin, N, Hin, Win, cin), p[pre + "conv1.weight"].shape))
-                dX = ops.conv3x3_dx(dz1, ops.conv_wflip(w1, planes, cin), Hin, Win, res=None if ds is not None else dres)
+                wf1 = ops.conv_wflip(w1, planes, cin)
+                dX = ops.conv3x3_dx(dz1, wf1, Hin, Win, res=None if ds is not None else dres, planes=_planes(wf1))
             else:
                 wgrad(pre + "conv1.weight", lambda: _w2d_grad(_conv3x3_dw(dz1, Xin, N, Hin, Win, cin, stride), p[pre + "conv1.weight"].shape))
                 dcol1 = ops.linear_dx(dz1, w1)
diff --git a/tailored-avsr_amd/tavsr/ops/__init__.py b/tailored-avsr_amd/tavsr/ops/__init__.py
--- a/tailored-avsr_amd/tavsr/ops/__init__.py
+++ b/tailored-avsr_amd/tavsr/ops/__init__.py
@@ -40,6 +40,7 @@
 CONV_TAPSKIP_STRIDE2 = os.environ.get("TAVSR_CONV_TAPSKIP_STRIDE2", "1") != "0"
 CONV_TAPSKIP_STRIDE2_DW = os.environ.get("TAVSR_CONV_TAPSKIP_STRIDE2_DW", "0") != "0"
 CONV_TAPSKIP_STRIDE2_MAXPOS = 36
+CONV_X6 = os.environ.get("TAVSR_CONV_X6", "1") != "0"
 
 CTC_ALIGN_CHUNK = 16
 
diff --git a/tailored-avsr_amd/tavsr/ops/vision.py b/tailored-avsr_amd/tavsr/ops/vision.py
--- a/tailored-avsr_amd/tavsr/ops/vision.py
+++ b/tailored-avsr_amd/tavsr/ops/vision.py
@@ -10,7 +10,7 @@
 __all__ = ["conv1_fwd", "conv1_bwd", "im2col3x3s2", "col2im3x3s2_relu", "conv_out", "im2col2d", "col2im2d", "stem_implicit_ok",
            "stem_pad16_ok", "stem_pad", "stem_weight_288", "stem_weight_grad_from_288", "stem_conv_fwd_pad16", "stem_conv_dw_pad16",
            "stem_conv_fwd", "stem_conv_dw", "im2col_stem", "bn_stats", "rsqrt_eps", "bn_apply_fwd", "bn_bwd", "bn_bwd_pooled",
-           "maxpool3x3s2_fwd", "bn_act_maxpool3x3s2_fwd", "maxpool3x3s2_bwd", "avgpool_fwd", "avgpool_bwd", "conv_wflip", "_tapskip",
+           "maxpool3x3s2_fwd", "bn_act_maxpool3x3s2_fwd", "maxpool3x3s2_bwd", "avgpool_fwd", "avgpool_bwd", "conv_wflip", "conv_wsplit", "x6_takes", "_tapskip",
            "_tapskip2", "_tapskip_any", "conv3x3_fwd", "conv3x3_dx", "conv3x3_dw"]
 
 
@@ -228,6 +228,25 @@
     return out
 
 
+def conv_wsplit(w):
+    require_cuda(w)
+    N, K = w.shape
+    assert w.stride(1) == 1 and K % 16 == 0
+    out = empty(5 * N * K // 2, like=w)
+    check(lib().tavsr_conv_wsplit(ptr(w), w.stride(0), ptr(out), N, K, stream()), "tavsr_conv_wsplit")
+    return out
+
+
+def x6_takes(w, taps=9, pad0=False):
+    return bool(ops.CONV_X6 and not pad0 and w.stride(1) == 1 and w.shape[1] % 32 == 0 and (taps == 9 or w.shape[1] >= 256))
+
+
+def _x6(w, planes, taps=9, pad0=False):
+    if not x6_takes(w, taps, pad0):
+        return w, 0
+    return (conv_wsplit(w) if planes is None else planes), 16
+
+
 def _tapskip_bits():
     return 1 | (0 if ops.CONV_TILEORDER else 2) | (0 if ops.CONV_DW_UNEVEN else 4)
 
@@ -246,7 +265,7 @@
     return _tapskip2(H, W, dw) if stride == 2 and taps == 9 and not pad0 else _tapskip(H, W, stride, taps, pad0, dw)
 
 
-def conv3x3_fwd(x, w2d, H, W, stride=1, taps=9, pad0=False, bias=None, act=None):
+def conv3x3_fwd(x, w2d, H, W, stride=1, taps=9, pad0=False, bias=None, act=None, planes=None):
     M, cin = x.shape
     cout = w2d.shape[0]
     if pad0:
@@ -256,16 +275,18 @@
         Ho, Wo = (H - 1) // stride + 1, (W - 1) // stride + 1
     Mo = M // (H * W) * Ho * Wo
     z = empty(Mo, cout, like=x)
-    gemm(Mo, cout, taps * cin, x, cin, w2d, taps * cin, z, cout, conv=(1, H, W, cin, stride, 90 if pad0 else taps, _tapskip_any(H, W, stride, taps, pad0)),
+    B, x6 = _x6(w2d, planes, taps, pad0)
+    gemm(Mo, cout, taps * cin, x, cin, B, taps * cin, z, cout, conv=(1, H, W, cin, stride, 90 if pad0 else taps, _tapskip_any(H, W, stride, taps, pad0) | x6),
          bias=bias, act=act)
     return z
 
 
-def conv3x3_dx(dz, wflip, H, W, res=None):
+def conv3x3_dx(dz, wflip, H, W, res=None, planes=None):
     M, cout = dz.shape
     cin = wflip.shape[0]
     dx = empty(M, cin, like=dz)
-    gemm(M, cin, 9 * cout, dz, cout, wflip, 9 * cout, dx, cin, conv=(1, H, W, cout, 0, 0, _tapskip(H, W)), R=res, ldr=0 if res is None else cin)
+    B, x6 = _x6(wflip, planes)
+    gemm(M, cin, 9 * cout, dz, cout, B, 9 * cout, dx, cin, conv=(1, H, W, cout, 0, 0, _tapskip(H, W) | x6), R=res, ldr=0 if res is None else cin)
     return dx
 
 
```

New measurement: 452.6 (median of 6 runs). +9.8%, better.
